# sanderslab/magellanmapper

Measured on AMD Instinct MI355X. Metric: Mvoxels/s, 2048x2048x1024 uint16 stack, 5-sigma LoG blob detection, higher is better.
Workload: dtype f16x2 MFMA (f32 accumulate) + 16-bit fixed-point intermediates; f64 re-score of every candidate

## Files before the change

include/mmx.h:

```cpp
#ifndef MMX_H
#define MMX_H

#include <stddef.h>
#include <stdint.h>

#ifdef __cplusplus
extern "C" {
#endif

#define MMX_ABI_VERSION 21

typedef enum {
    MMX_OK = 0,
    MMX_ERR_ARG = 1,
    MMX_ERR_HIP = 2,
    MMX_ERR_NO_DEVICE = 3,
    MMX_ERR_WORKSPACE = 4,
    MMX_ERR_UNSUPPORTED = 5,
    MMX_DEFERRED = 6
} mmx_status;

typedef enum { MMX_U8 = 0, MMX_U16 = 1, MMX_F32 = 2, MMX_F64 = 3 } mmx_dtype;

#define MMX_MAX_RADIUS_FAST 24
#define MMX_MAX_RADIUS_WIDE 64
#define MMX_MAX_RADIUS_GENERIC 255
#define MMX_MAX_BLOCKS 65535
#define MMX_COLOC_BALL 33

typedef struct {
    int64_t src_off;
    int32_t nz, ny, nx;
    int32_t slot;
    int32_t px;
    int32_t _pad;
} mmx_block;
#define MMX_ROW_ALIGN 32

typedef struct {
    const void* d_data;
    int32_t dtype;
    float value_range;
    int64_t stride_z, stride_y, stride_x;
} mmx_volume;

typedef struct {
    int32_t slot;
    int32_t s;
    int32_t z, y, x;
    uint32_t flags;
    float v;
    float nbr_max;
    double v64;
    uint64_t band;
} mmx_cand;

#define MMX_CAND_CONTESTED 1u
#define MMX_CAND_BAND 2u
#define MMX_CAND_PROBE 4u

int mmx_abi_version(void);
const char* mmx_strerror(int status);
const char* mmx_last_hip_error(void);
int mmx_device_count(void);

typedef enum {
    MMX_ZX_AUTO = -1,
    MMX_ZX_SEPARATE = 0,
    MMX_ZX_PACKED = 2,
    MMX_ZX_TILED = 6,
    MMX_ZX_TILED_Q16 = 7,
    MMX_ZX_WIDE = 8,
    MMX_ZX_THIN = 9
} mmx_zx_mode;
#define MMX_ZX_PREPACKED 0x100
#define MMX_ZX_Y_VALU    0x200
#define MMX_MASK_ROWS 1
#define MMX_MASK_QUADS 2
int mmx_log_batch_f32(const mmx_volume* vol, const mmx_block* d_blocks, const mmx_block* h_blocks,
                      int n_blocks, int64_t slot_elems,
                      const double* h_w0, const double* h_w2, int radius, double norm,
                      float* d_log, float* d_work, uint64_t* d_nms_mask, float nms_lo, float nms_eps,
                      int* h_mask_written, int zx_mode, int* h_zx_path, void* stream);

#define MMX_LOG_ABS_TOL 1e-4

double mmx_tiled_q16_error_bound(const double* h_w0, const double* h_w2, int radius, double norm);

#define MMX_COL_PREFETCH 4
#define MMX_FOLD_MAX_N 68
int mmx_fold_matrix(const float* w, int radius, int n, float* out );
int mmx_col_prefetch(void);

int mmx_zx_pack(const mmx_volume* vol, const mmx_block* d_blocks, const mmx_block* h_blocks, int n_blocks,
                int64_t slot_elems, float* d_work, void* stream);

size_t mmx_workspace_bytes(int n_blocks, int64_t slot_elems, int n_sigma, int with_masks);

int mmx_log_batch_f32_generic(const mmx_volume* vol, const mmx_block* d_blocks,
                              const mmx_block* h_blocks, int n_blocks, int64_t slot_elems,
                              const double* h_w0, const double* h_w2, int radius, double norm,
                              float* d_log, float* d_work, void* stream);

int mmx_peaks_batch(const float* d_log, const uint64_t* d_nms_mask, int mask_layout, int n_sigma, const mmx_block* d_blocks,
                    const mmx_block* h_blocks, int n_blocks, int64_t slot_elems,
                    float thr, float eps, mmx_cand* d_cands, uint32_t cap,
                    uint32_t* d_count, void* stream);

int mmx_rescore_f64(const mmx_volume* vol, const mmx_block* d_blocks, int n_blocks,
                    mmx_cand* d_pts, uint32_t cap, const uint32_t* d_count,
                    const double* d_w0, const double* d_w2, const int32_t* h_radius,
                    const double* h_norm, int n_sigma, int store_f32, void* stream);

int mmx_expand_probes(mmx_cand* d_cands, uint32_t cap, uint32_t* d_count, uint32_t* d_n_cands,
                      const mmx_block* d_blocks, int n_blocks, int n_sigma, void* stream);

typedef struct {
    int32_t parent;
    int32_t off[3];
    int32_t core_lo[3];
    int32_t core_hi[3];
} mmx_part;
int mmx_fold_parts(mmx_cand* d_cands, uint32_t cap, uint32_t* d_count, const mmx_part* d_parts, int n_parts,
                   void* stream);

typedef struct {
    const mmx_volume* vol32;
    const mmx_volume* vol_exact;
    const mmx_block* d_blocks;
    const mmx_block* h_blocks;
    int32_t n_blocks, n_sigma;
    int64_t slot_elems;
    const double* h_w0; const double* h_w2;
    const double* d_w0; const double* d_w2;
    const int32_t* h_radius;
    const double* h_norm;
    float* d_work;
    size_t work_bytes;
    float thr, eps;
    mmx_cand* d_cands;
    uint32_t cap, h_prefix;
    uint32_t* d_count;
    uint32_t* h_count;
    mmx_cand* h_cands;
    int32_t zx_mode, zx_flags, store_f32, exact, expand, _pad;
    void* stream; void* tail_stream; void* pack_stream;
    void* ev_work_free; void* ev_work_read; void* ev_done;
    const mmx_part* d_parts;
    const mmx_block* d_parents;
    const mmx_block* h_parents;
    int32_t n_parts, n_parents;
} mmx_detect_args;
typedef struct {
    int32_t zx_path;
    int32_t mask_layout;
    int32_t n_pass_rounds;
    int32_t _pad;
    double q16_bound;
} mmx_detect_info;
int mmx_detect_batch(const mmx_detect_args* args, mmx_detect_info* info);
const char* mmx_detect_last_error(void);
int mmx_log_scales_f32(const mmx_detect_args* args, mmx_detect_info* info);
int mmx_detect_batch_capture(const mmx_detect_args* args, mmx_detect_info* info, void** graph);
int mmx_graph_launch(void* graph, void* stream, void* ev_done, mmx_detect_info* info);
int mmx_graph_destroy(void* graph);
int mmx_event_synchronize(void* ev);
int mmx_stream_wait_event(void* stream, void* ev);
int mmx_timing_is_enabled(void);

int mmx_overlap_pairs(const double* d_blobs, const int32_t* d_offsets, int n_blocks,
                      double overlap, double band, double max_sigma, int32_t* d_pairs, double* d_frac,
                      uint32_t cap, uint32_t* d_count, void* stream);

int mmx_close_pairs(const int32_t* d_master, int n_master, const int32_t* d_check, int n_check,
                    const int32_t tol[3], int32_t* d_last, uint8_t* d_hit, void* stream);

typedef struct {
    int64_t src_off;
    int64_t dst_off;
    int64_t scratch_off;
    int32_t nz, ny, nx;
    int32_t qclass;
} mmx_subblock;

typedef struct {
    int32_t lo_prev, lo_next, hi_prev, hi_next;
    double lo_gamma, hi_gamma;
} mmx_quantile_class;

typedef struct {
    double clip_min, clip_max;
    double max_thresh;
    double unsharp_strength;
    double erosion_threshold;
    int32_t radius;
    int32_t rgb_guess;
    double tv_weight;
    double tv_factor;
} mmx_preproc_params;

#define MMX_PP_IDENTITY 1
#define MMX_PP_ERODED 2
#define MMX_PP_EXACT_MEAN 4
typedef struct {
    double vmin, vmax, mean;
    int32_t flags;
    int32_t _pad;
} mmx_subblock_info;

#define MMX_PP_RADIUS 32
#define MMX_PP_MAX_SIDE 32
#define MMX_PP_MAX_LDS 163840

int64_t mmx_preprocess_fast_lds(int nz, int ny, int nx);

int mmx_preprocess_batch(const mmx_volume* vol, const mmx_subblock* d_subs, const mmx_subblock* h_subs,
                         int n_subs, const mmx_quantile_class* d_qclasses, int n_qclasses,
                         const mmx_preproc_params* params, const double* d_weights,
                         int64_t dst_sy, int64_t dst_sz, float* d_out32, double* d_out64,
                         mmx_subblock_info* d_info, void* stream);

#define MMX_PP_AUTO 0
#define MMX_PP_SINGLE 1
#define MMX_PP_PIPELINED 2
#define MMX_PP_TILES_PER_WG 8
int64_t mmx_preprocess_work_bytes(const mmx_subblock* h_subs, int n_subs);
int mmx_preprocess_batch_mode(const mmx_volume* vol, const mmx_subblock* d_subs, const mmx_subblock* h_subs,
                              int n_subs, const mmx_quantile_class* d_qclasses, int n_qclasses,
                              const mmx_preproc_params* params, const double* d_weights,
                              int64_t dst_sy, int64_t dst_sz, float* d_out32, double* d_out64,
                              mmx_subblock_info* d_info, int mode, int tiles_per_wg,
                              void* d_work, int64_t work_bytes, void* stream);

int mmx_preprocess_batch_generic(const mmx_volume* vol, const mmx_subblock* d_subs,
                                 const mmx_subblock* h_subs, int n_subs,
                                 const mmx_quantile_class* d_qclasses, int n_qclasses,
                                 const mmx_preproc_params* params, const double* d_weights,
                                 int64_t dst_sy, int64_t dst_sz, float* d_out32, double* d_out64,
                                 mmx_subblock_info* d_info, double* d_scratch, int64_t scratch_doubles,
                                 void* stream);

int mmx_coloc_means(const mmx_volume* vol, const mmx_block* d_blocks, int n_blocks,
                    const int32_t* d_blobs, const int32_t* d_offsets, int n_blobs,
                    double* d_mean, int32_t* d_count, void* stream);
int mmx_coloc_voxels(const mmx_volume* vol, const mmx_block* d_blocks, int n_blocks,
                     const int32_t* d_blobs, const int32_t* d_offsets, int n_blobs,
                     double* d_mean, int32_t* d_count, double* d_voxels, void* stream);

int mmx_unmix_batch(const mmx_volume* vol, const mmx_volume* h_subs, const double* h_facs, int n_subs,
                    const mmx_block* d_blocks, const mmx_block* h_blocks, int n_blocks,
                    int64_t dst_slot, int64_t dst_sy, int64_t dst_sz,
                    float* d_out32, double* d_out64, void* stream);

typedef struct {
    int64_t src_off;
    int32_t in_nz, in_ny, in_nx;
    int32_t out_nz, out_ny, out_nx;
    int32_t slot;
    int32_t tz, ty, tx;
} mmx_resize_block;
int mmx_minmax_batch(const mmx_volume* vol, const mmx_block* d_blocks, const mmx_block* h_blocks,
                     int n_blocks, double* d_minmax, void* stream);
int mmx_resize_batch(const mmx_volume* vol, const mmx_resize_block* d_blocks,
                     const mmx_resize_block* h_blocks, int n_blocks,
                     const int32_t* d_index, const double* d_weight, const double* d_minmax,
                     int64_t dst_slot, int64_t dst_sy, int64_t dst_sz,
                     void* d_out, float* d_out32, void* stream);

int mmx_resize_batch_as(const mmx_volume* vol, const mmx_resize_block* d_blocks,
                        const mmx_resize_block* h_blocks, int n_blocks,
                        const int32_t* d_index, const double* d_weight, const double* d_minmax,
                        int64_t dst_slot, int64_t dst_sy, int64_t dst_sz,
                        int out_dtype, void* d_out, float* d_out32, void* stream);

int mmx_gauss_axis_batch(const mmx_volume* vol, const mmx_block* d_blocks, const mmx_block* h_blocks,
                         int n_blocks, int axis, const double* d_weights, const int32_t* d_radius,
                         int w_pitch, int nearest, int64_t dst_slot, int64_t dst_sy, int64_t dst_sz,
                         void* d_out, void* stream);

typedef struct { int32_t z0, z1; int64_t rank[4]; } mmx_rank_group;
size_t mmx_order_stats_workspace(int n_groups);
int mmx_order_stats(const mmx_volume* vol, int64_t nz, int64_t ny, int64_t nx,
                    const mmx_rank_group* d_groups, const mmx_rank_group* h_groups, int n_groups,
                    double* d_stats , int32_t* d_nan ,
                    void* d_work, size_t work_bytes, void* stream);

#define MMX_K_COUNT 14
#define MMX_K_THIN 14
#define MMX_K_SLOTS 15
int mmx_timing_enable(int on);
int mmx_timing_read(double* ms, int64_t* launches, int n);

int mmx_copy_rect_h2d(void* d_dst, size_t dpitch, const void* h_src, size_t spitch, size_t width, size_t height,
                      void* stream);
int mmx_host_stage_upload(const void* h_src, void* d_dst, const int64_t* regions, int32_t n_regions, int64_t nz,
                          int64_t ny, int64_t row_bytes, void* const* h_staging, int64_t staging_bytes, int32_t depth,
                          void* const* events, void* stream, int32_t device, int64_t* n_queued, const int32_t* cancel,
                          int32_t n_threads);
int mmx_host_stage_upload_pitched(const void* h_src, int64_t src_pitch, void* d_dst, const int64_t* regions,
                                  int32_t n_regions, int64_t nz, int64_t ny, int64_t row_bytes, void* const* h_staging,
                                  int64_t staging_bytes, int32_t depth, void* const* events, void* stream, int32_t device,
                                  int64_t* n_queued, const int32_t* cancel, int32_t n_threads);
int mmx_event_query(void* ev);
int mmx_event_create(void** ev);
int mmx_event_destroy(void* ev);
int mmx_event_record(void* ev, void* stream);
int mmx_event_elapsed_ms(void* start, void* stop, float* ms);

int mmx_host_prune_axis(const int32_t* zyx, const int32_t* tag, double* abs_zyx,
                        const int64_t* cur, int64_t n_cur, int axis, int n_sections,
                        const double* bounds, double last_end, const int32_t tol[3],
                        const double* nxt_lo, const double* nxt_hi,
                        int64_t* out_cur, int64_t* out_n,
                        int64_t* n_slab, int64_t* n_after, int64_t* n_next);

typedef struct {
    const int32_t* src_cols;
    int64_t n_out, n_main;
    int32_t abs_dst[3];
} mmx_row_layout;
int mmx_host_take_rows(const double* table, int64_t ld, const int64_t* rows, int64_t n, const double* abs_zyx,
                       const mmx_row_layout* layout, double* out, double* out_rest);
int mmx_host_gather_parts_by_key(const double* table, int64_t ld, int32_t n_parts, const int64_t* const* ids,
                                 const int64_t* const* keys, const double* const* abs_rows, const int64_t* n_rows,
                                 int64_t n_keys, const mmx_row_layout* layout, double* out, int64_t out_rows,
                                 double* out_rest);

int mmx_host_prune_region(const int32_t* zyx, const int32_t* tag, double* abs_zyx, const int64_t* cur, int64_t n_cur,
                          int64_t own_lo, int64_t own_hi, const int32_t n_sections[3], const double* const bounds[3],
                          const double last_end[3], const int32_t tol[3], const double* const nxt_lo[3],
                          const double* const nxt_hi[3], int64_t* out_rows, int64_t* out_keys, int64_t* out_n,
                          int64_t* n_slab, int64_t* n_after, int64_t* n_next, int64_t stat_ld);
int mmx_host_prune_parts(const int32_t* zyx, const int32_t* tag, const double* abs_zyx, const double* chan,
                         int64_t chan_ld, const int64_t* parts, int n_parts, int own_part, const int32_t box_lo[3],
                         const int32_t box_hi[3], const double* channels, int n_channels,
                         const int32_t n_sections[3], const double* const bounds[3], const double last_end[3],
                         const int32_t tol[3], const double* const nxt_lo[3], const double* const nxt_hi[3],
                         int64_t n_keys, int64_t* out_ids, int64_t* out_keys, double* out_abs, int64_t* out_n,
                         int64_t* n_slab, int64_t* n_after, int64_t* n_next, int64_t stat_ld);
int mmx_host_rows_in_boxes(const int32_t* zyx, const int32_t* tag, const double* abs_zyx, const double* chan,
                           int64_t chan_ld, int64_t n, const int32_t* box_lo, const int32_t* box_hi, int n_boxes,
                           double* out, int64_t cap, int64_t* out_n);
int mmx_host_append_rows(const double* payload, int64_t n, const int32_t lo[3], const int32_t hi[3], int32_t* zyx,
                         int32_t* tag, double* abs_zyx, double* chan, int64_t chan_ld, int64_t at, int64_t cap,
                         int64_t* out_n);
int mmx_host_emit_parts(const double* table, int64_t ld, int32_t n_parts, const int64_t* const* ids,
                        const int64_t* const* keys, const double* const* abs_rows, const int64_t* n_rows,
                        const mmx_row_layout* layout, double* out, int64_t out_rows);
int mmx_host_merge_parts_by_key(const double* const* parts, const int64_t* n_rows, int32_t n_parts, int64_t ld,
                                int64_t n_keys, int64_t n_cols, double* out, int64_t out_rows);

int mmx_host_map_columns(const double* table, int64_t ld, int64_t n, const int32_t* src_cols,
                         int32_t n_map, double* out, int64_t out_ld, int32_t dst_col0);

int mmx_host_resolve_peaks(const mmx_cand* cands, uint32_t n_cands, uint32_t n_total, const mmx_block* blocks,
                           int n_blocks, int n_sigma, double thr, int32_t* out_nz_coords, double* out_nz_vals,
                           int32_t* out_coords, double* out_vals, int32_t* offsets, uint8_t* ties, double* stats);
int mmx_host_overlap_prune(const int32_t* coords, const int32_t* offsets, int n_blocks, const double* sigmas,
                           int n_sigma, double overlap, double band, uint8_t* alive, uint8_t* open_blocks,
                           int32_t* pairs, double* frac, int64_t cap, int64_t* n_pairs, int64_t* n_knife);
int mmx_host_emit_tables(const int32_t* coords, const uint8_t* alive, const int32_t* offsets, int n_blocks,
                         const double* sigmas, int n_sigma, double channel, const double* block_offsets,
                         const int32_t* block_tags, const int32_t* interior, double* store, int64_t ld,
                         int32_t* zyx, int32_t* tag, double* abs_zyx, int64_t row0, int64_t capacity,
                         int64_t* rows_per_block);
int mmx_host_emit_tables_multi(int32_t n_channels, const int32_t* const* coords, const uint8_t* const* alive,
                               const int32_t* const* offsets, int n_blocks, const double* const* sigmas,
                               const int32_t* n_sigma, const double* channel_ids, const double* block_offsets,
                               const int32_t* block_tags, const int32_t* interior, double* store, int64_t ld,
                               int32_t n_extra, int32_t* zyx, int32_t* tag, double* abs_zyx, int64_t row0,
                               int64_t capacity, int64_t* rows_per_block, uint8_t* any_before, int32_t* coloc_rows);
int mmx_host_coloc_flags(const double* means, const int32_t* mean_channels, int32_t n_mean_channels, int64_t n,
                         const int32_t* rows, const int64_t* row_offsets, int n_blocks, const int32_t* shapes,
                         int32_t n_channels, double* flags, int64_t ld);

typedef struct {
    const mmx_cand* cands; uint32_t n_cands, n_total;
    const mmx_block* blocks; int32_t n_blocks, n_sigma;
    double thr, eps;
    const double* sigmas; double overlap, overlap_band;
    double channel;
    const double* block_offsets; const int32_t* block_tags; const int32_t* interior;
    double* store; int64_t ld; int32_t* zyx; int32_t* tag; double* abs_zyx; int64_t capacity;
    int64_t* rows_per_block; uint8_t* any_before;
    const int32_t* n_sections; const double* const* bounds; const double* last_end; const int32_t* tol;
    const double* const* nxt_lo; const double* const* nxt_hi;
    int64_t* n_slab; int64_t* n_after; int64_t* n_next; int64_t stat_ld;
    const int32_t* src_cols; int32_t n_out, abs_dst0;
    double* out; int64_t out_capacity; int64_t* out_rows;
    double* stats;
} mmx_finish_stack_args;
int mmx_host_finish_stack(const mmx_finish_stack_args* a);

int mmx_cdist_f64(const double* d_a, int64_t n, const double* d_b, int64_t m, int dim, double* d_out, void* stream);
int mmx_host_lsap(const double* cost, int64_t nr, int64_t nc, int64_t* out_rows, int64_t* out_cols);

#define MMX_PATCH_MAX_SIZE 4096
int mmx_extract_patches(const mmx_volume* vol, const int32_t* d_zyx, int64_t n, int size, void* d_out, float* d_out32,
                        void* stream);

int mmx_calib_stream(int kind, const void* d_in, void* d_out, int64_t n_elems, void* stream);

#ifdef __cplusplus
}
#endif
#endif
```

magellanmapper_amd/_native.py:

```python
from __future__ import annotations

import ctypes
import os
from ctypes import (POINTER, Structure, c_char_p, c_double, c_float, c_int, c_int32, c_int64,
                    c_uint8, c_uint32, c_void_p)

import numpy as np

_HERE = os.path.dirname(os.path.abspath(__file__))
LIB_PATH = os.environ.get("MMX_LIB_PATH") or os.path.join(_HERE, "libmmx_hip.so")

MMX_ABI_VERSION = 21
MMX_U8, MMX_U16, MMX_F32, MMX_F64 = 0, 1, 2, 3
MMX_MAX_RADIUS_FAST = 24
MMX_MAX_RADIUS_WIDE = 64
MMX_MAX_RADIUS_GENERIC = 255
MMX_CAND_CONTESTED = 1
MMX_CAND_BAND = 2
MMX_CAND_PROBE = 4
MMX_ZX_AUTO, MMX_ZX_SEPARATE, MMX_ZX_PACKED, MMX_ZX_MFMA_F32, MMX_ZX_MFMA_F16, MMX_ZX_MFMA_F16_LDS = -1, 0, 2, 3, 4, 5
MMX_ZX_TILED, MMX_ZX_TILED_Q16, MMX_ZX_PREPACKED, MMX_ZX_Y_VALU = 6, 7, 0x100, 0x200
MMX_ZX_WIDE = 8
MMX_ZX_THIN = 9
MMX_FOLD_MAX_N = 68
MMX_MASK_ROWS, MMX_MASK_QUADS = 1, 2
MMX_MAX_BLOCKS = 65535
MMX_COLOC_BALL = 33
MMX_PATCH_MAX_SIZE = 4096

BLOCK_DTYPE = np.dtype([("src_off", "<i8"), ("nz", "<i4"), ("ny", "<i4"), ("nx", "<i4"),
                        ("slot", "<i4"), ("px", "<i4"), ("_pad", "<i4")], align=True)
MMX_ROW_ALIGN = 32
CAND_DTYPE = np.dtype([("slot", "<i4"), ("s", "<i4"), ("z", "<i4"), ("y", "<i4"), ("x", "<i4"),
                       ("flags", "<u4"), ("v", "<f4"), ("nbr_max", "<f4"), ("v64", "<f8"),
                       ("band", "<u8")], align=True)
assert BLOCK_DTYPE.itemsize == 32 and CAND_DTYPE.itemsize == 48
PART_DTYPE = np.dtype([("parent", "<i4"), ("off", "<i4", (3,)), ("core_lo", "<i4", (3,)), ("core_hi", "<i4", (3,))],
                      align=True)
assert PART_DTYPE.itemsize == 40
SUBBLOCK_DTYPE = np.dtype([("src_off", "<i8"), ("dst_off", "<i8"), ("scratch_off", "<i8"),
                           ("nz", "<i4"), ("ny", "<i4"), ("nx", "<i4"), ("qclass", "<i4")], align=True)
QCLASS_DTYPE = np.dtype([("lo_prev", "<i4"), ("lo_next", "<i4"), ("hi_prev", "<i4"), ("hi_next", "<i4"),
                         ("lo_gamma", "<f8"), ("hi_gamma", "<f8")], align=True)
SUBINFO_DTYPE = np.dtype([("vmin", "<f8"), ("vmax", "<f8"), ("mean", "<f8"), ("flags", "<i4"),
                          ("_pad", "<i4")], align=True)
assert SUBBLOCK_DTYPE.itemsize == 40 and QCLASS_DTYPE.itemsize == 32 and SUBINFO_DTYPE.itemsize == 32
MMX_PP_IDENTITY, MMX_PP_ERODED, MMX_PP_EXACT_MEAN = 1, 2, 4
MMX_PP_AUTO, MMX_PP_SINGLE, MMX_PP_PIPELINED = 0, 1, 2
RESIZE_DTYPE = np.dtype([("src_off", "<i8"), ("in_nz", "<i4"), ("in_ny", "<i4"), ("in_nx", "<i4"),
                         ("out_nz", "<i4"), ("out_ny", "<i4"), ("out_nx", "<i4"), ("slot", "<i4"),
                         ("tz", "<i4"), ("ty", "<i4"), ("tx", "<i4")], align=True)
assert RESIZE_DTYPE.itemsize == 48
RANK_GROUP_DTYPE = np.dtype([("z0", "<i4"), ("z1", "<i4"), ("rank", "<i8", (4,))], align=True)
assert RANK_GROUP_DTYPE.itemsize == 40


class Volume(Structure):
    _fields_ = [("d_data", c_void_p), ("dtype", c_int32), ("value_range", c_float),
                ("stride_z", c_int64), ("stride_y", c_int64), ("stride_x", c_int64)]


class DetectArgs(Structure):
    _fields_ = [("vol32", POINTER(Volume)), ("vol_exact", POINTER(Volume)), ("d_blocks", c_void_p),
                ("h_blocks", c_void_p), ("n_blocks", c_int32), ("n_sigma", c_int32), ("slot_elems", c_int64),
                ("h_w0", c_void_p), ("h_w2", c_void_p), ("d_w0", c_void_p), ("d_w2", c_void_p),
                ("h_radius", c_void_p), ("h_norm", c_void_p), ("d_work", c_void_p), ("work_bytes", ctypes.c_size_t),
                ("thr", c_float), ("eps", c_float), ("d_cands", c_void_p), ("cap", c_uint32), ("h_prefix", c_uint32),
                ("d_count", c_void_p), ("h_count", c_void_p), ("h_cands", c_void_p),
                ("zx_mode", c_int32), ("zx_flags", c_int32), ("store_f32", c_int32), ("exact", c_int32),
                ("expand", c_int32), ("_pad", c_int32),
                ("stream", c_void_p), ("tail_stream", c_void_p), ("pack_stream", c_void_p),
                ("ev_work_free", c_void_p), ("ev_work_read", c_void_p), ("ev_done", c_void_p),
                ("d_parts", c_void_p), ("d_parents", c_void_p), ("h_parents", c_void_p),
                ("n_parts", c_int32), ("n_parents", c_int32)]


class FinishStackArgs(Structure):
    _fields_ = [("cands", c_void_p), ("n_cands", c_uint32), ("n_total", c_uint32),
                ("blocks", c_void_p), ("n_blocks", c_int32), ("n_sigma", c_int32),
                ("thr", c_double), ("eps", c_double),
                ("sigmas", c_void_p), ("overlap", c_double), ("overlap_band", c_double),
                ("channel", c_double),
                ("block_offsets", c_void_p), ("block_tags", c_void_p), ("interior", c_void_p),
                ("store", c_void_p), ("ld", c_int64), ("zyx", c_void_p), ("tag", c_void_p), ("abs_zyx", c_void_p),
                ("capacity", c_int64), ("rows_per_block", c_void_p), ("any_before", c_void_p),
                ("n_sections", c_void_p), ("bounds", c_void_p), ("last_end", c_void_p), ("tol", c_void_p),
                ("nxt_lo", c_void_p), ("nxt_hi", c_void_p),
                ("n_slab", c_void_p), ("n_after", c_void_p), ("n_next", c_void_p), ("stat_ld", c_int64),
                ("src_cols", c_void_p), ("n_out", c_int32), ("abs_dst0", c_int32),
                ("out", c_void_p), ("out_capacity", c_int64), ("out_rows", c_void_p),
                ("stats", c_void_p)]


MMX_DEFERRED = 6


class RowLayout(Structure):
    _fields_ = [("src_cols", POINTER(c_int32)), ("n_out", c_int64), ("n_main", c_int64), ("abs_dst", c_int32 * 3)]


class DetectInfo(Structure):
    _fields_ = [("zx_path", c_int32), ("mask_layout", c_int32), ("n_pass_rounds", c_int32), ("_pad", c_int32),
                ("q16_bound", c_double)]


class PreprocParams(Structure):
    _fields_ = [("clip_min", c_double), ("clip_max", c_double), ("max_thresh", c_double),
                ("unsharp_strength", c_double), ("erosion_threshold", c_double),
                ("radius", c_int32), ("rgb_guess", c_int32), ("tv_weight", c_double), ("tv_factor", c_double)]


class MmxError(RuntimeError):
    """A C-ABI call returned a non-zero status."""


_lib = None

SYMBOLS = (
    "mmx_abi_version", "mmx_strerror", "mmx_last_hip_error", "mmx_device_count",
    "mmx_detect_batch", "mmx_log_scales_f32", "mmx_detect_batch_capture", "mmx_graph_launch", "mmx_graph_destroy", "mmx_detect_last_error",
    "mmx_event_synchronize", "mmx_stream_wait_event", "mmx_timing_is_enabled",
    "mmx_log_batch_f32", "mmx_log_batch_f32_generic", "mmx_zx_pack", "mmx_fold_matrix", "mmx_col_prefetch", "mmx_tiled_q16_error_bound", "mmx_workspace_bytes", "mmx_peaks_batch", "mmx_rescore_f64",
    "mmx_overlap_pairs", "mmx_close_pairs", "mmx_event_create", "mmx_event_destroy",
    "mmx_event_record", "mmx_event_elapsed_ms", "mmx_timing_enable", "mmx_timing_read",
    "mmx_calib_stream", "mmx_host_prune_axis",
    "mmx_preprocess_fast_lds", "mmx_preprocess_batch", "mmx_preprocess_batch_mode", "mmx_preprocess_work_bytes", "mmx_preprocess_batch_generic",
    "mmx_coloc_means", "mmx_coloc_voxels", "mmx_host_take_rows", "mmx_host_map_columns", "mmx_resize_batch_as", "mmx_gauss_axis_batch", "mmx_unmix_batch", "mmx_minmax_batch", "mmx_resize_batch",
    "mmx_cdist_f64", "mmx_host_lsap", "mmx_expand_probes", "mmx_fold_parts", "mmx_host_resolve_peaks", "mmx_host_overlap_prune",
    "mmx_host_emit_tables", "mmx_host_prune_region", "mmx_host_prune_parts", "mmx_host_rows_in_boxes", "mmx_host_append_rows", "mmx_host_emit_parts", "mmx_host_merge_parts_by_key", "mmx_host_gather_parts_by_key", "mmx_host_emit_tables_multi", "mmx_host_coloc_flags", "mmx_host_finish_stack", "mmx_copy_rect_h2d", "mmx_host_stage_upload", "mmx_host_stage_upload_pitched", "mmx_event_query",
    "mmx_order_stats_workspace", "mmx_order_stats", "mmx_extract_patches",
)
KERNEL_KINDS = ("zpass", "ypass", "xpass", "generic", "peaks", "rescore", "overlap_pairs",
                "close_pairs", "zxpass", "y2pass", "preproc", "coloc", "zxpack", "widepass")
MORE_KERNEL_KINDS = ("thinpass",)
_ALL_KINDS = KERNEL_KINDS + MORE_KERNEL_KINDS


def lib() -> ctypes.CDLL:
    global _lib
    if _lib is not None:
        return _lib
    if not os.path.exists(LIB_PATH):
        raise MmxError(
            f"{LIB_PATH} not found: the HIP extension has not been built "
            "(run __graft_entry__.build() or make -C magellanmapper_amd/csrc). "
            "There is no CPU fallback for this path.")
    try:
        import torch
    except ImportError:
        pass
    L = ctypes.CDLL(LIB_PATH)
    missing = [name for name in SYMBOLS if not hasattr(L, name)]
    if missing:
        raise MmxError(f"{LIB_PATH} lacks {', '.join(missing)}: it was built from older sources; rebuild it")
    vp = c_void_p
    L.mmx_abi_version.restype = c_int
    L.mmx_strerror.restype = c_char_p
    L.mmx_strerror.argtypes = [c_int]
    L.mmx_last_hip_error.restype = c_char_p
    L.mmx_device_count.restype = c_int
    log_args = [POINTER(Volume), vp, vp, c_int, c_int64, POINTER(c_double), POINTER(c_double),
                c_int, c_double, vp, vp]
    L.mmx_log_batch_f32.argtypes = log_args + [vp, c_float, c_float, POINTER(c_int), c_int, POINTER(c_int), vp]
    L.mmx_log_batch_f32_generic.argtypes = log_args + [vp]
    L.mmx_workspace_bytes.argtypes = [c_int, c_int64, c_int, c_int]
    L.mmx_workspace_bytes.restype = ctypes.c_size_t
    L.mmx_zx_pack.argtypes = [POINTER(Volume), vp, vp, c_int, c_int64, vp, vp]
    L.mmx_tiled_q16_error_bound.argtypes = [POINTER(c_double), POINTER(c_double), c_int, c_double]
    L.mmx_tiled_q16_error_bound.restype = c_double
    L.mmx_fold_matrix.argtypes = [POINTER(c_float), c_int, c_int, POINTER(c_float)]
    L.mmx_fold_matrix.restype = c_int
    L.mmx_col_prefetch.argtypes = []
    L.mmx_col_prefetch.restype = c_int
    L.mmx_peaks_batch.argtypes = [vp, vp, c_int, c_int, vp, vp, c_int, c_int64, c_float, c_float, vp,
                                  c_uint32, vp, vp]
    L.mmx_rescore_f64.argtypes = [POINTER(Volume), vp, c_int, vp, c_uint32, vp, vp, vp,
                                  POINTER(c_int32), POINTER(c_double), c_int, c_int, vp]
    L.mmx_overlap_pairs.argtypes = [vp, vp, c_int, c_double, c_double, c_double, vp, vp, c_uint32, vp, vp]
    L.mmx_close_pairs.argtypes = [vp, c_int, vp, c_int, POINTER(c_int32), vp, vp, vp]
    L.mmx_detect_batch.argtypes = [POINTER(DetectArgs), POINTER(DetectInfo)]
    L.mmx_log_scales_f32.argtypes = [POINTER(DetectArgs), POINTER(DetectInfo)]
    L.mmx_detect_batch_capture.argtypes = [POINTER(DetectArgs), POINTER(DetectInfo), POINTER(vp)]
    L.mmx_graph_launch.argtypes = [vp, vp, vp, POINTER(DetectInfo)]
    L.mmx_graph_destroy.argtypes = [vp]
    L.mmx_detect_last_error.restype = c_char_p
    L.mmx_event_synchronize.argtypes = [vp]
    L.mmx_stream_wait_event.argtypes = [vp, vp]
    L.mmx_event_create.argtypes = [POINTER(vp)]
    L.mmx_event_destroy.argtypes = [vp]
    L.mmx_event_record.argtypes = [vp, vp]
    L.mmx_event_elapsed_ms.argtypes = [vp, vp, POINTER(c_float)]
    L.mmx_timing_enable.argtypes = [c_int]
    L.mmx_timing_read.argtypes = [POINTER(c_double), POINTER(c_int64), c_int]
    L.mmx_calib_stream.argtypes = [c_int, vp, vp, c_int64, vp]
    L.mmx_host_prune_axis.argtypes = [vp, vp, vp, vp, c_int64, c_int, c_int, vp, c_double,
                                      POINTER(c_int32), vp, vp, vp, POINTER(c_int64), vp, vp, vp]
    L.mmx_preprocess_fast_lds.argtypes = [c_int, c_int, c_int]
    L.mmx_preprocess_fast_lds.restype = c_int64
    pre_args = [POINTER(Volume), vp, vp, c_int, vp, c_int, POINTER(PreprocParams), vp,
                c_int64, c_int64, vp, vp, vp]
    L.mmx_preprocess_batch.argtypes = pre_args + [vp]
    L.mmx_preprocess_batch_mode.argtypes = pre_args + [c_int, c_int, vp, c_int64, vp]
    L.mmx_preprocess_work_bytes.argtypes = [vp, c_int]
    L.mmx_preprocess_work_bytes.restype = c_int64
    L.mmx_preprocess_batch_generic.argtypes = pre_args + [vp, c_int64, vp]
    L.mmx_minmax_batch.argtypes = [POINTER(Volume), vp, vp, c_int, vp, vp]
    L.mmx_minmax_batch.restype = c_int
    L.mmx_resize_batch.argtypes = [POINTER(Volume), vp, vp, c_int, vp, vp, vp, c_int64, c_int64, c_int64,
                                   vp, vp, vp]
    L.mmx_resize_batch.restype = c_int
    L.mmx_resize_batch_as.argtypes = [POINTER(Volume), vp, vp, c_int, vp, vp, vp, c_int64, c_int64, c_int64,
                                      c_int, vp, vp, vp]
    L.mmx_resize_batch_as.restype = c_int
    L.mmx_gauss_axis_batch.argtypes = [POINTER(Volume), vp, vp, c_int, c_int, vp, vp, c_int, c_int,
                                       c_int64, c_int64, c_int64, vp, vp]
    L.mmx_gauss_axis_batch.restype = c_int
    L.mmx_unmix_batch.argtypes = [POINTER(Volume), POINTER(Volume), POINTER(c_double), c_int, vp, vp, c_int,
                                  c_int64, c_int64, c_int64, vp, vp, vp]
    L.mmx_unmix_batch.restype = c_int
    L.mmx_host_take_rows.argtypes = [vp, c_int64, vp, c_int64, vp, POINTER(RowLayout), vp, vp]
    L.mmx_host_map_columns.argtypes = [vp, c_int64, c_int64, POINTER(c_int32), c_int32, vp, c_int64, c_int32]
    L.mmx_cdist_f64.argtypes = [vp, c_int64, vp, c_int64, c_int, vp, vp]
    L.mmx_cdist_f64.restype = c_int
    L.mmx_host_lsap.argtypes = [vp, c_int64, c_int64, vp, vp]
    L.mmx_host_lsap.restype = c_int
    L.mmx_coloc_means.argtypes = [POINTER(Volume), vp, c_int, vp, vp, c_int, vp, vp, vp]
    L.mmx_coloc_means.restype = c_int
    L.mmx_coloc_voxels.argtypes = [POINTER(Volume), vp, c_int, vp, vp, c_int, vp, vp, vp, vp]
    L.mmx_coloc_voxels.restype = c_int
    L.mmx_expand_probes.argtypes = [vp, c_uint32, vp, vp, vp, c_int, c_int, vp]
    L.mmx_expand_probes.restype = c_int
    L.mmx_fold_parts.argtypes = [vp, c_uint32, vp, vp, c_int, vp]
    L.mmx_fold_parts.restype = c_int
    L.mmx_host_resolve_peaks.argtypes = [vp, c_uint32, c_uint32, vp, c_int, c_int, c_double, vp, vp, vp, vp, vp, vp, vp]
    L.mmx_host_overlap_prune.argtypes = [vp, vp, c_int, vp, c_int, c_double, c_double, vp, vp, vp, vp, c_int64,
                                         POINTER(c_int64), POINTER(c_int64)]
    L.mmx_host_prune_region.argtypes = [vp, vp, vp, vp, c_int64, c_int64, c_int64, POINTER(c_int32), POINTER(vp),
                                        POINTER(c_double), POINTER(c_int32), POINTER(vp), POINTER(vp), vp, vp,
                                        POINTER(c_int64), vp, vp, vp, c_int64]
    L.mmx_host_prune_parts.argtypes = [vp, vp, vp, vp, c_int64, vp, c_int, c_int, POINTER(c_int32), POINTER(c_int32),
                                       vp, c_int, POINTER(c_int32), POINTER(vp), POINTER(c_double), POINTER(c_int32),
                                       POINTER(vp), POINTER(vp), c_int64, vp, vp, vp, POINTER(c_int64), vp, vp, vp,
                                       c_int64]
    L.mmx_host_rows_in_boxes.argtypes = [vp, vp, vp, vp, c_int64, c_int64, vp, vp, c_int, vp, c_int64, POINTER(c_int64)]
    L.mmx_host_append_rows.argtypes = [vp, c_int64, POINTER(c_int32), POINTER(c_int32), vp, vp, vp, vp, c_int64,
                                       c_int64, c_int64, POINTER(c_int64)]
    L.mmx_host_gather_parts_by_key.argtypes = [vp, c_int64, c_int32, vp, vp, vp, vp, c_int64, POINTER(RowLayout), vp, c_int64, vp]
    L.mmx_host_emit_parts.argtypes = [vp, c_int64, c_int32, vp, vp, vp, vp, POINTER(RowLayout), vp, c_int64]
    L.mmx_host_merge_parts_by_key.argtypes = [vp, vp, c_int32, c_int64, c_int64, c_int64, vp, c_int64]
    L.mmx_host_emit_tables_multi.argtypes = [c_int32, vp, vp, vp, c_int, vp, vp, vp, vp, vp, vp, vp, c_int64, c_int32, vp, vp,
                                             vp, c_int64, c_int64, vp, vp, vp]
    L.mmx_host_coloc_flags.argtypes = [vp, vp, c_int32, c_int64, vp, vp, c_int, vp, c_int32, vp, c_int64]
    L.mmx_host_finish_stack.argtypes = [POINTER(FinishStackArgs)]
    L.mmx_host_stage_upload.argtypes = [vp, vp, vp, c_int32, c_int64, c_int64, c_int64, vp, c_int64, c_int32, vp, vp, c_int32,
                                        vp, vp, c_int32]
    L.mmx_host_stage_upload_pitched.argtypes = [vp, c_int64, vp, vp, c_int32, c_int64, c_int64, c_int64, vp, c_int64, c_int32,
                                                vp, vp, c_int32, vp, vp, c_int32]
    L.mmx_event_query.argtypes = [vp]
    L.mmx_copy_rect_h2d.argtypes = [vp, ctypes.c_size_t, vp, ctypes.c_size_t, ctypes.c_size_t, ctypes.c_size_t, vp]
    L.mmx_host_emit_tables.argtypes = [vp, vp, vp, c_int, vp, c_int, c_double, vp, vp, vp, vp, c_int64, vp, vp, vp,
                                       c_int64, c_int64, vp]
    L.mmx_order_stats_workspace.argtypes = [c_int]
    L.mmx_order_stats_workspace.restype = ctypes.c_size_t
    L.mmx_order_stats.argtypes = [POINTER(Volume), c_int64, c_int64, c_int64, vp, vp, c_int, vp, vp, vp, ctypes.c_size_t, vp]
    L.mmx_order_stats.restype = c_int
    L.mmx_extract_patches.argtypes = [POINTER(Volume), vp, c_int64, c_int, vp, vp, vp]
    L.mmx_extract_patches.restype = c_int
    L.mmx_preprocess_batch.restype = c_int
    L.mmx_preprocess_batch_mode.restype = c_int
    L.mmx_preprocess_batch_generic.restype = c_int
    for name in SYMBOLS:
        fn = getattr(L, name)
        if name in ("mmx_preprocess_fast_lds", "mmx_workspace_bytes", "mmx_preprocess_work_bytes",
                    "mmx_order_stats_workspace"):
            continue
        if fn.restype is None or name.startswith(("mmx_log", "mmx_peaks", "mmx_rescore",
                                                  "mmx_overlap", "mmx_close", "mmx_event", "mmx_timing", "mmx_calib", "mmx_host")):
            fn.restype = c_int
    if L.mmx_abi_version() != MMX_ABI_VERSION:
        raise MmxError("libmmx_hip.so ABI version mismatch")
    _lib = L
    return L


def check(status: int, what: str) -> None:
    if status != 0:
        L = lib()
        msg = L.mmx_strerror(status).decode()
        hip = L.mmx_last_hip_error().decode()
        raise MmxError(f"{what}: {msg}" + (f" ({hip})" if hip else ""))


def as_double_ptr(a: np.ndarray):
    assert a.dtype == np.float64 and a.flags.c_contiguous
    return a.ctypes.data_as(POINTER(c_double))


def as_int32_ptr(a: np.ndarray):
    assert a.dtype == np.int32 and a.flags.c_contiguous
    return a.ctypes.data_as(POINTER(c_int32))


def timing_enable(on: bool = True, kinds=None) -> None:
    mask = 1 if on else 0
    if on and kinds is not None:
        mask = 0
        for k in kinds:
            mask |= 1 << (_ALL_KINDS.index(k) + 1)
    check(lib().mmx_timing_enable(mask), "mmx_timing_enable")


def timing_read() -> dict:
    ms = (c_double * len(_ALL_KINDS))()
    n = (c_int64 * len(_ALL_KINDS))()
    check(lib().mmx_timing_read(ms, n, len(_ALL_KINDS)), "mmx_timing_read")
    return {k: (ms[i], n[i]) for i, k in enumerate(_ALL_KINDS)}


def col_prefetch() -> int:
    return int(lib().mmx_col_prefetch())


def fold_matrix(w: np.ndarray, n: int) -> np.ndarray:
    w = np.ascontiguousarray(w, dtype=np.float32)
    out = np.empty((int(n), int(n)), dtype=np.float32)
    check(lib().mmx_fold_matrix(w.ctypes.data_as(POINTER(c_float)), len(w) - 1, int(n),
                                out.ctypes.data_as(POINTER(c_float))), "mmx_fold_matrix")
    return out


def keep_host_heap(mmap_threshold: int = 1 << 30, trim_threshold: int = (1 << 31) - 1) -> bool:
    try:
        libc = ctypes.CDLL("libc.so.6")
        ok1 = libc.mallopt(-3, int(mmap_threshold))
        ok2 = libc.mallopt(-1, int(trim_threshold))
        return bool(ok1 and ok2)
    except (OSError, AttributeError):
        return False
```

magellanmapper_amd/csrc/mmx_api.hip:

```cpp

#include <atomic>
#include <cstdio>
#include <cstdlib>
#include <cstring>

#include "mmx_common.h"

int mmx_launch_generic_pass(int pass, const mmx_volume* vol, const mmx_block* d_blocks, int n_blocks,
                            int max_vox, int64_t slot_elems, const float* w0, const float* w2, int radius,
                            const float* in1, const float* in2, float* out1, float* out2, hipStream_t s);
int mmx_launch_fold_pass(int pass, const mmx_volume* vol, const mmx_block* d_blocks, int n_blocks,
                         int max_vox, int64_t slot_elems, const float* w0, const float* w2, int radius,
                         const float* in1, const float* in2, float* out1, float* out2, hipStream_t s);
int mmx_launch_peaks(const float* d_log, int n_sigma, int64_t sigma_stride, const mmx_block* d_blocks,
                     int n_blocks, int max_vox, int64_t slot_elems, float thr, float eps,
                     mmx_cand* d_cands, uint32_t cap, uint32_t* d_count, hipStream_t stream);
int mmx_launch_peaks_sparse(const float* d_log, const unsigned long long* d_mask, int n_sigma,
                            int64_t sigma_stride, const mmx_block* d_blocks, int n_blocks, int max_vox,
                            int64_t slot_elems, float thr, float eps, mmx_cand* d_cands, uint32_t cap,
                            uint32_t* d_count, int quads, hipStream_t stream);

#include <mutex>
#include <vector>

namespace {
thread_local char g_hip_err[256] = "";

struct span { hipEvent_t a, b; int kind; };
std::mutex g_tm;
bool g_timing = false;
uint32_t g_kinds = ~0u;
std::vector<span> g_spans;
std::vector<hipEvent_t> g_pool;
hipEvent_t g_open[MMX_K_SLOTS];

hipEvent_t take_event()
{
    if (!g_pool.empty()) { hipEvent_t e = g_pool.back(); g_pool.pop_back(); return e; }
    hipEvent_t e = nullptr;
    hipEventCreate(&e);
    return e;
}

int hip_fail(hipError_t e, const char* what)
{
    snprintf(g_hip_err, sizeof g_hip_err, "%s: %s", what, hipGetErrorString(e));
    return MMX_ERR_HIP;
}
}

void mmx_time_begin(int kind, hipStream_t s)
{
    std::lock_guard<std::mutex> lk(g_tm);
    if (!g_timing || !((g_kinds >> kind) & 1u)) return;
    g_open[kind] = take_event();
    hipEventRecord(g_open[kind], s);
}

void mmx_time_end(int kind, hipStream_t s)
{
    std::lock_guard<std::mutex> lk(g_tm);
    if (!g_timing || !g_open[kind]) return;
    hipEvent_t b = take_event();
    hipEventRecord(b, s);
    g_spans.push_back({g_open[kind], b, kind});
    g_open[kind] = nullptr;
}

extern "C" {

int mmx_timing_enable(int on)
{
    std::lock_guard<std::mutex> lk(g_tm);
    for (auto& sp : g_spans) { g_pool.push_back(sp.a); g_pool.push_back(sp.b); }
    g_spans.clear();
    for (int k = 0; k < MMX_K_SLOTS; ++k) g_open[k] = nullptr;
    g_timing = on != 0;
    g_kinds = on == 1 ? ~0u : ((uint32_t)on >> 1);
    return MMX_OK;
}

int mmx_timing_is_enabled(void)
{
    std::lock_guard<std::mutex> lk(g_tm);
    return g_timing ? 1 : 0;
}

int mmx_timing_read(double* ms, int64_t* launches, int n)
{
    if (!ms || !launches || n < MMX_K_COUNT) return MMX_ERR_ARG;
    std::lock_guard<std::mutex> lk(g_tm);
    for (int k = 0; k < n; ++k) { ms[k] = 0.0; launches[k] = 0; }
    for (auto& sp : g_spans) {
        if (sp.kind >= n) {
            g_pool.push_back(sp.a);
            g_pool.push_back(sp.b);
            continue;
        }
        hipError_t r = hipEventSynchronize(sp.b);
        if (r != hipSuccess) return hip_fail(r, "hipEventSynchronize");
        float t = 0.f;
        r = hipEventElapsedTime(&t, sp.a, sp.b);
        if (r != hipSuccess) return hip_fail(r, "hipEventElapsedTime");
        ms[sp.kind] += t;
        launches[sp.kind] += 1;
        g_pool.push_back(sp.a);
        g_pool.push_back(sp.b);
    }
    g_spans.clear();
    return MMX_OK;
}

int mmx_abi_version(void) { return MMX_ABI_VERSION; }
size_t mmx_workspace_bytes(int n_blocks, int64_t slot_elems, int n_sigma, int with_masks)
{
    if (n_blocks < 1 || slot_elems < 1 || n_sigma < 1) return 0;
    size_t bytes = (size_t)(4 + n_sigma) * (size_t)n_blocks * (size_t)slot_elems * sizeof(float);
    if (with_masks) {
        bytes = (bytes + 15) & ~(size_t)15;
        bytes += (size_t)n_sigma * (((size_t)n_blocks * (size_t)slot_elems) >> 5) * 16;
    }
    return bytes;
}

const char* mmx_strerror(int status)
{
    switch (status) {
        case MMX_OK: return "ok";
        case MMX_ERR_ARG: return "bad argument";
        case MMX_ERR_HIP: return "HIP runtime error";
        case MMX_ERR_NO_DEVICE: return "no gfx950 device";
        case MMX_ERR_WORKSPACE: return "workspace too small";
        case MMX_ERR_UNSUPPORTED: return "unsupported configuration";
        case MMX_DEFERRED: return "left to the caller";
        default: return "unknown status";
    }
}

const char* mmx_last_hip_error(void) { return g_hip_err; }


int mmx_device_count(void)
{
    int n = 0;
    hipError_t e = hipGetDeviceCount(&n);
    if (e != hipSuccess) { hip_fail(e, "hipGetDeviceCount"); return -1; }
    int ok = 0;
    for (int i = 0; i < n; ++i) {
        hipDeviceProp_t p;
        if (hipGetDeviceProperties(&p, i) == hipSuccess && strncmp(p.gcnArchName, "gfx950", 6) == 0) ++ok;
    }
    return ok;
}

double mmx_tiled_q16_error_bound(const double* h_w0, const double* h_w2, int radius, double norm)
{
    return mmx_q16_error_bound(h_w0, h_w2, radius, norm);
}

}

void mmx_batch_geom_make(const mmx_volume* vol, const mmx_block* h_blocks, int n_blocks, int64_t slot_elems,
                         mmx_batch_geom* g)
{
    *g = mmx_batch_geom{};
    g->min_nz = g->min_ny = g->min_nx = 1 << 30;
    g->plan_status = MMX_ERR_UNSUPPORTED;
    g->rows_fit = g->quads_fit = true;
    if (n_blocks < 1 || n_blocks > MMX_MAX_BLOCKS) {
        g->status = n_blocks < 1 ? MMX_ERR_ARG : MMX_ERR_UNSUPPORTED;
        return;
    }
    for (int i = 0; i < n_blocks; ++i) {
        const mmx_block& b = h_blocks[i];
        if (b.nz < 1 || b.ny < 1 || b.nx < 1 || b.slot != i || b.px < b.nx || b.px % MMX_ROW_ALIGN) {
            if (g->status == MMX_OK) g->status = MMX_ERR_ARG;
            g->bad_block = true;
            return;
        }
        if ((int64_t)b.nz * b.ny * b.px > slot_elems && g->status == MMX_OK) g->status = MMX_ERR_WORKSPACE;
        if (b.nz < g->min_nz) g->min_nz = b.nz;
        if (b.ny < g->min_ny) g->min_ny = b.ny;
        if (b.nx < g->min_nx) g->min_nx = b.nx;
        if (b.ny > g->max_ny) g->max_ny = b.ny;
        if (b.nx > g->max_nx) g->max_nx = b.nx;
        if (b.px > g->max_px) g->max_px = b.px;
        if (b.ny * b.px > g->max_zcols) g->max_zcols = b.ny * b.px;
        if (b.nz * b.px > g->max_ycols) g->max_ycols = b.nz * b.px;
        if (b.nz * b.ny > g->max_rows) g->max_rows = b.nz * b.ny;
        if (b.nz * b.ny * b.px > g->max_vox) g->max_vox = b.nz * b.ny * b.px;
        if (!mmx_entries_fit(MMX_MASK_ROWS, b.nz, b.ny, b.nx, b.px, slot_elems)) g->rows_fit = false;
        if (!mmx_entries_fit(MMX_MASK_QUADS, b.nz, b.ny, b.nx, b.px, slot_elems)) g->quads_fit = false;
        if (vol) {
            const int64_t lane = (int64_t)(b.ny - 1) * vol->stride_y + (int64_t)(b.nx - 1) * vol->stride_x;
            if (lane > g->max_lane_in) g->max_lane_in = lane;
        }
    }
    if (vol) g->plan_status = mmx_zx6_plan_make(h_blocks, n_blocks, slot_elems, vol->dtype, &g->plan);
}

namespace {

struct pass_weights {
    float z0[MMX_MAX_RADIUS_GENERIC + 1], z2[MMX_MAX_RADIUS_GENERIC + 1];
    float y0[MMX_MAX_RADIUS_GENERIC + 1], y2[MMX_MAX_RADIUS_GENERIC + 1];
    float x0[MMX_MAX_RADIUS_GENERIC + 1], x2[MMX_MAX_RADIUS_GENERIC + 1];
};
void make_weights(const mmx_volume* vol, const double* h_w0, const double* h_w2, int radius, double norm, pass_weights* w)
{
    double in_scale = 1.0;
    if (vol->dtype == MMX_U8) in_scale = 1.0 / 255.0;
    else if (vol->dtype == MMX_U16) in_scale = 1.0 / 65535.0;
    for (int k = 0; k <= radius; ++k) {
        w->z0[k] = (float)(h_w0[k] * in_scale);
        w->z2[k] = (float)(h_w2[k] * in_scale);
        w->y0[k] = (float)h_w0[k];
        w->y2[k] = (float)h_w2[k];
        w->x0[k] = (float)(-norm * h_w0[k]);
        w->x2[k] = (float)(-norm * h_w2[k]);
    }
}
mmx_taps_f32 taps(const float* a, const float* b, int radius)
{
    mmx_taps_f32 t;
    for (int k = 0; k <= MMX_MAX_RADIUS_FAST; ++k) {
        t.w0[k] = k <= radius ? a[k] : 0.f;
        t.w2[k] = k <= radius ? b[k] : 0.f;
    }
    return t;
}

int launched(int rc, const char* launcher, const char* what)
{
    if (rc == MMX_ERR_HIP) return hip_fail(hipGetLastError(), what);
    if (rc == MMX_ERR_UNSUPPORTED) {
        char msg[128];
        snprintf(msg, sizeof msg, "%s refused a call its route accepted", launcher);
        mmx_detect_set_error(msg);
    }
    return rc;
}

struct pass_scope {
    int kind; hipStream_t s;
    pass_scope(int k, hipStream_t st) : kind(k), s(st) { if (k >= 0) mmx_time_begin(k, st); }
    ~pass_scope() { if (kind >= 0) mmx_time_end(kind, s); }
};

int fused_passes(const mmx_log_call& c, const mmx_route& r, const mmx_batch_geom& g, const pass_weights& w)
{
    const mmx_volume* vol = c.vol;
    const int radius = c.radius, n_blocks = c.n_blocks;
    const int64_t slot_elems = c.slot_elems;
    hipStream_t s = c.stream;
    float* t0 = c.d_work;
    float* t1 = c.d_work + (int64_t)n_blocks * slot_elems;
    mmx_taps_f32 tzz = taps(w.z0, w.z2, radius), txx = taps(w.y0, w.y2, radius), tyy = taps(w.x0, w.x2, radius);
    const bool tiled = r.family == MMX_ROUTE_TILED;
    const mmx_zx6_plan& plan = g.plan;
    int rc;
    if (r.makes_copy) {
        mmx_timed_scope ts(MMX_K_ZXPACK, s);
        rc = mmx_launch_zx6_pack(vol, c.d_blocks, c.h_blocks, n_blocks, plan, c.d_work, s);
        if (rc != MMX_OK) return launched(rc, "mmx_launch_zx6_pack", "voxel copy of the tiled path");
    }
    { mmx_timed_scope ts(MMX_K_ZX, s);
      if (tiled)
          rc = mmx_launch_zx6(vol, c.d_blocks, c.h_blocks, n_blocks, plan, txx, radius, c.d_work,
                              r.q16 ? (float)(1.0 / r.bp) : 0.f, r.q16 ? (float)(1.0 / r.bq) : 0.f, s);
      else
          rc = mmx_launch_zx2(vol, c.d_blocks, n_blocks, g.max_ny, g.max_px, slot_elems, tzz, txx, radius, t0, t1, s); }
    if (rc != MMX_OK) return launched(rc, tiled ? "mmx_launch_zx6" : "mmx_launch_zx2", "fused passes");
    { mmx_timed_scope ts(MMX_K_Y2, s);
      unsigned long long* d_mask = r.layout ? (unsigned long long*)c.d_nms_mask : nullptr;
      const float cp = r.q16 ? (float)(r.bp / 65535.0) : 0.f, cq = r.q16 ? (float)(r.bq / 32767.0) : 0.f;
      if (r.y_kernel == MMX_Y_YM)
          rc = mmx_launch_ym(c.d_blocks, n_blocks, plan, slot_elems, tyy, radius, c.d_work, cp, cq, c.d_log, d_mask,
                             c.nms_lo, c.nms_eps, s);
      else if (r.y_kernel == MMX_Y_Y6)
          rc = mmx_launch_y6(c.d_blocks, n_blocks, plan, slot_elems, tyy, radius, c.d_work,
                             reinterpret_cast<const float*>(reinterpret_cast<const char*>(c.d_work) + plan.q_off), cp, cq,
                             c.d_log, d_mask, c.nms_lo, c.nms_eps, s);
      else
          rc = mmx_launch_y2(c.d_blocks, n_blocks, g.max_ycols, slot_elems, tyy, radius, t0, t1, c.d_log, d_mask, c.nms_lo,
                             c.nms_eps, s); }
    return launched(rc, r.y_kernel == MMX_Y_YM ? "mmx_launch_ym" : (r.y_kernel == MMX_Y_Y6 ? "mmx_launch_y6" : "mmx_launch_y2"),
                    "fused passes");
}

int wide_passes(const mmx_log_call& c, const mmx_route& r, const pass_weights& w)
{
    const int radius = c.radius, n_blocks = c.n_blocks;
    const int64_t slot_elems = c.slot_elems;
    hipStream_t s = c.stream;
    float* t0 = c.d_work;
    float* t1 = t0 + (int64_t)n_blocks * slot_elems;
    float* t2 = t1 + (int64_t)n_blocks * slot_elems;
    float* t3 = t2 + (int64_t)n_blocks * slot_elems;
    unsigned long long* d_mask = r.layout ? (unsigned long long*)c.d_nms_mask : nullptr;
    int rc;
    { mmx_timed_scope ts(MMX_K_WIDE, s);
      rc = mmx_launch_wide_pass(0, c.vol, c.d_blocks, c.h_blocks, n_blocks, slot_elems, w.z0, w.z2, radius, nullptr, nullptr,
                                t2, t3, nullptr, 0.f, 0.f, s); }
    if (rc == MMX_OK) {
        mmx_timed_scope ts(MMX_K_WIDE, s);
        rc = mmx_launch_wide_pass(1, c.vol, c.d_blocks, c.h_blocks, n_blocks, slot_elems, w.y0, w.y2, radius, t2, t3, t0, t1,
                                  nullptr, 0.f, 0.f, s);
    }
    if (rc == MMX_OK) {
        mmx_timed_scope ts(MMX_K_WIDE, s);
        rc = mmx_launch_wide_pass(2, c.vol, c.d_blocks, c.h_blocks, n_blocks, slot_elems, w.x0, w.x2, radius, t0, t1, c.d_log,
                                  nullptr, d_mask, c.nms_lo, c.nms_eps, s);
    }
    return launched(rc, "mmx_launch_wide_pass", "wide passes");
}

int three_passes(const mmx_volume* vol, const mmx_block* d_blocks, int n_blocks, int64_t slot_elems, int radius,
                 float* d_work, float* d_log, const mmx_batch_geom& g, const pass_weights& w, int rings, int folds,
                 bool timed, hipStream_t s)
{
    float* t0 = d_work;
    float* t1 = t0 + (int64_t)n_blocks * slot_elems;
    float* t2 = t1 + (int64_t)n_blocks * slot_elems;
    float* t3 = t2 + (int64_t)n_blocks * slot_elems;
    const float* w0[3] = {w.z0, w.y0, w.x0};
    const float* w2[3] = {w.z2, w.y2, w.x2};
    const float* in1[3] = {nullptr, t0, t2};
    const float* in2[3] = {nullptr, t1, t3};
    float* out1[3] = {t0, t2, d_log};
    float* out2[3] = {t1, t3, nullptr};
    const int ring_kind[3] = {MMX_K_ZPASS, MMX_K_YPASS, MMX_K_XPASS};
    const char* ring_name[3] = {"mmx_launch_zpass", "mmx_launch_ypass", "mmx_launch_xpass"};
    const char* what[3] = {"z pass", "y pass", "x pass"};
    for (int p = 0; p < 3; ++p) {
        const bool ring = (rings >> p) & 1, fold = !ring && ((folds >> p) & 1);
        int rc;
        { pass_scope ts(!timed ? -1 : (ring ? ring_kind[p] : (fold ? MMX_K_THIN : MMX_K_GENERIC)), s);
        if (ring && p == 0) rc = mmx_launch_zpass(vol, d_blocks, n_blocks, g.max_zcols, slot_elems, taps(w.z0, w.z2, radius), radius, t0, t1, s);
        else if (ring && p == 1) rc = mmx_launch_ypass(d_blocks, n_blocks, g.max_ycols, slot_elems, taps(w.y0, w.y2, radius), radius, t0, t1, t2, t3, s);
        else if (ring) rc = mmx_launch_xpass(d_blocks, n_blocks, g.max_rows, g.max_nx, slot_elems, taps(w.x0, w.x2, radius), radius, t2, t3, d_log, s);
        else rc = (fold ? mmx_launch_fold_pass : mmx_launch_generic_pass)(p, vol, d_blocks, n_blocks, g.max_vox, slot_elems, w0[p], w2[p],
                                                                          radius, in1[p], in2[p], out1[p], out2[p], s); }
        if (rc != MMX_OK)
            return launched(rc, ring ? ring_name[p] : (fold ? "mmx_launch_fold_pass" : "mmx_launch_generic_pass"), what[p]);
    }
    return MMX_OK;
}

}

int mmx_log_scale_check(const mmx_log_call& c)
{
    mmx_zx_request q;
    if (mmx_zx_parse(c.zx_mode, &q) != MMX_OK) return MMX_ERR_ARG;
    if (!c.vol || !c.vol->d_data || !c.d_blocks || !c.h_blocks || !c.h_w0 || !c.h_w2 || !c.d_log || !c.d_work)
        return MMX_ERR_ARG;
    if (c.n_blocks < 1 || c.radius < 0 || c.slot_elems < 1) return MMX_ERR_ARG;
    if (c.n_blocks > MMX_MAX_BLOCKS) return MMX_ERR_UNSUPPORTED;
    if (c.radius > MMX_MAX_RADIUS_GENERIC) return MMX_ERR_UNSUPPORTED;
    if (c.slot_elems >= (int64_t(1) << 29)) return MMX_ERR_UNSUPPORTED;
    if (c.slot_elems % MMX_ROW_ALIGN) return MMX_ERR_ARG;
    if (!mmx_voxels_ok(c.vol)) return MMX_ERR_UNSUPPORTED;
    return MMX_OK;
}

int mmx_log_scale_run(const mmx_log_call& c, const mmx_batch_geom& g, const mmx_route& r)
{
    pass_weights w;
    make_weights(c.vol, c.h_w0, c.h_w2, c.radius, c.norm, &w);
    int rc;
    if (r.family == MMX_ROUTE_WIDE) rc = wide_passes(c, r, w);
    else if (r.family == MMX_ROUTE_SEPARATE)
        rc = three_passes(c.vol, c.d_blocks, c.n_blocks, c.slot_elems, c.radius, c.d_work, c.d_log, g, w,
                          r.ring_z | r.ring_y << 1 | r.ring_x << 2, r.fold_z | r.fold_y << 1 | r.fold_x << 2, true, c.stream);
    else rc = fused_passes(c, r, g, w);
    if (rc != MMX_OK) return rc;
    if (c.h_zx_path) *c.h_zx_path = r.path;
    if (c.h_mask_written) *c.h_mask_written = r.layout;
    return MMX_OK;
}

namespace {
int log_scale(const mmx_log_call& c, const mmx_batch_geom& g)
{
    if (c.h_mask_written) *c.h_mask_written = 0;
    if (c.h_zx_path) *c.h_zx_path = MMX_ZX_SEPARATE;
    int rc = mmx_log_scale_check(c);
    if (rc != MMX_OK) return rc;
    mmx_route r;
    rc = mmx_route_scale(c.vol, g, c.radius, c.h_w0, c.h_w2, c.norm, c.zx_mode, c.nms_eps, c.d_nms_mask && c.h_mask_written, &r);
    return rc != MMX_OK ? rc : mmx_log_scale_run(c, g, r);
}
}

int mmx_zx_pack_geom(const mmx_volume* vol, const mmx_block* d_blocks, const mmx_block* h_blocks, int n_blocks,
                     int64_t slot_elems, const mmx_batch_geom& g, float* d_work, hipStream_t stream)
{
    if (!vol || !vol->d_data || !d_blocks || !h_blocks || !d_work || n_blocks < 1 || slot_elems < 1) return MMX_ERR_ARG;
    if (n_blocks > MMX_MAX_BLOCKS) return MMX_ERR_UNSUPPORTED;
    if (vol->dtype != MMX_U8 && vol->dtype != MMX_U16 && vol->dtype != MMX_F32) return MMX_ERR_UNSUPPORTED;
    if (g.bad_block) return MMX_ERR_ARG;
    if (g.plan_status != MMX_OK) return g.plan_status;
    mmx_timed_scope ts(MMX_K_ZXPACK, stream);
    const int rc = mmx_launch_zx6_pack(vol, d_blocks, h_blocks, n_blocks, g.plan, d_work, stream);
    return rc == MMX_ERR_HIP ? hip_fail(hipGetLastError(), "voxel copy of the tiled path") : rc;
}

extern "C" {

int mmx_log_batch_f32(const mmx_volume* vol, const mmx_block* d_blocks, const mmx_block* h_blocks,
                      int n_blocks, int64_t slot_elems,
                      const double* h_w0, const double* h_w2, int radius, double norm,
                      float* d_log, float* d_work, uint64_t* d_nms_mask, float nms_lo, float nms_eps,
                      int* h_mask_written, int zx_mode, int* h_zx_path, void* stream)
{
    mmx_batch_geom g{};
    if (vol && h_blocks) mmx_batch_geom_make(vol, h_blocks, n_blocks, slot_elems, &g);
    return log_scale({vol, d_blocks, h_blocks, n_blocks, slot_elems, h_w0, h_w2, radius, norm, d_log, d_work,
                              d_nms_mask, nms_lo, nms_eps, h_mask_written, zx_mode, h_zx_path, (hipStream_t)stream}, g);
}

int mmx_log_batch_f32_generic(const mmx_volume* vol, const mmx_block* d_blocks, const mmx_block* h_blocks,
                              int n_blocks, int64_t slot_elems,
                              const double* h_w0, const double* h_w2, int radius, double norm,
                              float* d_log, float* d_work, void* stream)
{
    if (!vol || !vol->d_data || !d_blocks || !h_blocks || !h_w0 || !h_w2 || !d_log || !d_work)
        return MMX_ERR_ARG;
    if (n_blocks < 1 || radius < 0 || radius > MMX_MAX_RADIUS_GENERIC || slot_elems < 1) return MMX_ERR_ARG;
    if (n_blocks > MMX_MAX_BLOCKS) return MMX_ERR_UNSUPPORTED;
    mmx_batch_geom g;
    mmx_batch_geom_make(vol, h_blocks, n_blocks, slot_elems, &g);
    if (g.status != MMX_OK) return g.status;
    pass_weights w;
    make_weights(vol, h_w0, h_w2, radius, norm, &w);
    return three_passes(vol, d_blocks, n_blocks, slot_elems, radius, d_work, d_log, g, w, 0, 0, false, (hipStream_t)stream);
}

int mmx_zx_pack(const mmx_volume* vol, const mmx_block* d_blocks, const mmx_block* h_blocks, int n_blocks,
                int64_t slot_elems, float* d_work, void* stream)
{
    mmx_batch_geom g{};
    if (vol && h_blocks) mmx_batch_geom_make(vol, h_blocks, n_blocks, slot_elems, &g);
    return mmx_zx_pack_geom(vol, d_blocks, h_blocks, n_blocks, slot_elems, g, d_work, (hipStream_t)stream);
}

int mmx_peaks_batch(const float* d_log, const uint64_t* d_nms_mask, int mask_layout, int n_sigma, const mmx_block* d_blocks,
                    const mmx_block* h_blocks, int n_blocks, int64_t slot_elems,
                    float thr, float eps, mmx_cand* d_cands, uint32_t cap,
                    uint32_t* d_count, void* stream)
{
    if (!d_log || !d_blocks || !h_blocks || !d_cands || !d_count) return MMX_ERR_ARG;
    if (n_sigma < 1 || n_blocks < 1 || slot_elems < 1 || !(eps >= 0.f)) return MMX_ERR_ARG;
    if (n_blocks > MMX_MAX_BLOCKS) return MMX_ERR_UNSUPPORTED;
    if (slot_elems % MMX_ROW_ALIGN) return MMX_ERR_ARG;
    if (d_nms_mask && mask_layout != MMX_MASK_ROWS && mask_layout != MMX_MASK_QUADS) return MMX_ERR_ARG;
    mmx_batch_geom g;
    mmx_batch_geom_make(nullptr, h_blocks, n_blocks, slot_elems, &g);
    if (g.status != MMX_OK) return g.status;
    const int max_vox = g.max_vox;
    mmx_timed_scope ts(MMX_K_PEAKS, (hipStream_t)stream);
    int rc;
    if (d_nms_mask)
        rc = mmx_launch_peaks_sparse(d_log, (const unsigned long long*)d_nms_mask, n_sigma,
                                     (int64_t)n_blocks * slot_elems, d_blocks, n_blocks, max_vox, slot_elems,
                                     thr, eps, d_cands, cap, d_count, mask_layout == MMX_MASK_QUADS, (hipStream_t)stream);
    else
        rc = mmx_launch_peaks(d_log, n_sigma, (int64_t)n_blocks * slot_elems, d_blocks, n_blocks, max_vox,
                              slot_elems, thr, eps, d_cands, cap, d_count, (hipStream_t)stream);
    return rc == MMX_ERR_HIP ? hip_fail(hipGetLastError(), "peaks") : rc;
}

int mmx_copy_rect_h2d(void* d_dst, size_t dpitch, const void* h_src, size_t spitch, size_t width, size_t height,
                      void* stream)
{
    if (!d_dst || !h_src || width > dpitch || width > spitch) return MMX_ERR_ARG;
    if (!width || !height) return MMX_OK;
    hipError_t r = hipMemcpy2DAsync(d_dst, dpitch, h_src, spitch, width, height, hipMemcpyHostToDevice, (hipStream_t)stream);
    return r == hipSuccess ? MMX_OK : hip_fail(r, "hipMemcpy2DAsync");
}

int mmx_event_create(void** ev)
{
    if (!ev) return MMX_ERR_ARG;
    hipEvent_t e;
    hipError_t r = hipEventCreate(&e);
    if (r != hipSuccess) return hip_fail(r, "hipEventCreate");
    *ev = (void*)e;
    return MMX_OK;
}

int mmx_event_destroy(void* ev)
{
    hipError_t r = hipEventDestroy((hipEvent_t)ev);
    return r == hipSuccess ? MMX_OK : hip_fail(r, "hipEventDestroy");
}

int mmx_event_record(void* ev, void* stream)
{
    hipError_t r = hipEventRecord((hipEvent_t)ev, (hipStream_t)stream);
    return r == hipSuccess ? MMX_OK : hip_fail(r, "hipEventRecord");
}

int mmx_event_elapsed_ms(void* start, void* stop, float* ms)
{
    if (!ms) return MMX_ERR_ARG;
    hipError_t r = hipEventSynchronize((hipEvent_t)stop);
    if (r != hipSuccess) return hip_fail(r, "hipEventSynchronize");
    r = hipEventElapsedTime(ms, (hipEvent_t)start, (hipEvent_t)stop);
    return r == hipSuccess ? MMX_OK : hip_fail(r, "hipEventElapsedTime");
}

}
```

magellanmapper_amd/csrc/mmx_common.h:

```cpp
#pragma once

#include <hip/hip_runtime.h>
#include <stdint.h>

#include "../../include/mmx.h"

#define MMX_WG 256
#define MMX_MAX_GRID_X 2147483647

struct mmx_taps_f32 {
    float w0[MMX_MAX_RADIUS_FAST + 1];
    float w2[MMX_MAX_RADIUS_FAST + 1];
};

__host__ __device__ __forceinline__ int mmx_reflect(int i, int n)
{
    if (n == 1) return 0;
    const int period = 2 * n;
    i %= period;
    if (i < 0) i += period;
    return i < n ? i : period - 1 - i;
}

int mmx_launch_zpass(const mmx_volume* vol, const mmx_block* d_blocks, int n_blocks, int max_cols,
                     int64_t slot_elems, const mmx_taps_f32& taps, int radius,
                     float* d_gz, float* d_gzz, hipStream_t stream);
int mmx_launch_ypass(const mmx_block* d_blocks, int n_blocks, int max_cols, int64_t slot_elems,
                     const mmx_taps_f32& taps, int radius, const float* d_gz, const float* d_gzz,
                     float* d_a, float* d_bc, hipStream_t stream);
int mmx_launch_xpass(const mmx_block* d_blocks, int n_blocks, int max_rows, int max_nx,
                     int64_t slot_elems, const mmx_taps_f32& taps, int radius,
                     const float* d_a, const float* d_bc, float* d_log, hipStream_t stream);

int mmx_launch_zx2(const mmx_volume* vol, const mmx_block* d_blocks, int n_blocks, int max_ny, int max_px,
                   int64_t slot_elems, const mmx_taps_f32& tz, const mmx_taps_f32& tx, int radius,
                   float* d_p, float* d_q, hipStream_t s);
struct mmx_zx6_plan {
    int64_t tile_stride;
    int64_t pack_stride;
    int64_t q_off, tab_off, pack_off;
    int64_t tab_bytes;
    int max_tiles;
    int max_rowtiles;
};
int mmx_zx6_plan_make(const mmx_block* h_blocks, int n_blocks, int64_t slot_elems, int voxel_dtype, mmx_zx6_plan* plan);
int mmx_launch_zx6_pack(const mmx_volume* vol, const mmx_block* d_blocks, const mmx_block* h_blocks, int n_blocks,
                        const mmx_zx6_plan& plan, void* d_work, hipStream_t stream);
int mmx_launch_zx6(const mmx_volume* vol, const mmx_block* d_blocks, const mmx_block* h_blocks, int n_blocks,
                   const mmx_zx6_plan& plan, const mmx_taps_f32& tx, int radius, void* d_work, float qp, float qq,
                   hipStream_t stream);
int mmx_launch_y6(const mmx_block* d_blocks, int n_blocks, const mmx_zx6_plan& plan, int64_t slot_elems,
                  const mmx_taps_f32& taps, int radius, const float* d_p, const float* d_q, float cp, float cq,
                  float* d_log, unsigned long long* d_mask, float nms_lo, float nms_eps, hipStream_t stream);
int mmx_launch_ym(const mmx_block* d_blocks, int n_blocks, const mmx_zx6_plan& plan, int64_t slot_elems,
                  const mmx_taps_f32& taps, int radius, const float* d_p, float cp, float cq,
                  float* d_log, unsigned long long* d_mask, float nms_lo, float nms_eps, hipStream_t stream);
int mmx_launch_y2(const mmx_block* d_blocks, int n_blocks, int max_cols, int64_t slot_elems,
                  const mmx_taps_f32& taps, int radius, const float* d_p, const float* d_q,
                  float* d_log, unsigned long long* d_mask, float nms_lo, float nms_eps, hipStream_t stream);

int mmx_launch_wide_pass(int pass, const mmx_volume* vol, const mmx_block* d_blocks, const mmx_block* h_blocks, int n_blocks,
                         int64_t slot_elems, const float* w0, const float* w2, int radius,
                         const float* in1, const float* in2, float* out1, float* out2,
                         unsigned long long* d_mask, float nms_lo, float nms_eps, hipStream_t s);

struct mmx_batch_geom {
    int status;
    bool bad_block;
    int min_nz, min_ny, min_nx, max_ny, max_nx, max_px;
    int max_zcols, max_ycols, max_rows, max_vox;
    int64_t max_lane_in;
    bool rows_fit, quads_fit;
    mmx_zx6_plan plan;
    int plan_status;
};
void mmx_batch_geom_make(const mmx_volume* vol, const mmx_block* h_blocks, int n_blocks, int64_t slot_elems, mmx_batch_geom* g);

#include "mmx_entries.h"

#include "mmx_route.h"

struct mmx_log_call {
    const mmx_volume* vol; const mmx_block* d_blocks; const mmx_block* h_blocks; int n_blocks; int64_t slot_elems;
    const double* h_w0; const double* h_w2; int radius; double norm;
    float* d_log; float* d_work; uint64_t* d_nms_mask; float nms_lo, nms_eps; int* h_mask_written;
    int zx_mode; int* h_zx_path; hipStream_t stream;
};
int mmx_log_scale_check(const mmx_log_call& c);
int mmx_log_scale_run(const mmx_log_call& c, const mmx_batch_geom& g, const mmx_route& r);
int mmx_zx_pack_geom(const mmx_volume* vol, const mmx_block* d_blocks, const mmx_block* h_blocks, int n_blocks,
                     int64_t slot_elems, const mmx_batch_geom& g, float* d_work, hipStream_t stream);
void mmx_detect_set_error(const char* msg);

enum mmx_kernel_kind {
    MMX_K_ZPASS = 0, MMX_K_YPASS, MMX_K_XPASS, MMX_K_GENERIC, MMX_K_PEAKS, MMX_K_RESCORE,
    MMX_K_PAIRS, MMX_K_CLOSE, MMX_K_ZX, MMX_K_Y2, MMX_K_PREPROC, MMX_K_COLOC, MMX_K_ZXPACK, MMX_K_WIDE, MMX_K_END
};
void mmx_time_begin(int kind, hipStream_t s);
void mmx_time_end(int kind, hipStream_t s);
static_assert(MMX_K_END == MMX_K_COUNT, "kernel kinds out of sync with mmx.h");
static_assert(MMX_K_THIN == MMX_K_END && MMX_K_SLOTS == MMX_K_THIN + 1, "the thin family follows the counted ones");
struct mmx_timed_scope {
    int kind; hipStream_t s;
    mmx_timed_scope(int k, hipStream_t st) : kind(k), s(st) { mmx_time_begin(k, st); }
    ~mmx_timed_scope() { mmx_time_end(kind, s); }
};
```

magellanmapper_amd/csrc/mmx_fused4.hip:

```cpp

#include <algorithm>
#include <type_traits>

#include "mmx_device.h"

#define MMX_ZX4_MAXCLS 8
#ifndef ZX4_ST_AUX
#define ZX4_ST_AUX 0
#endif
#ifndef ZX4_LD_AUX
#define ZX4_LD_AUX 0
#endif

struct mmx_zx4_cfg {
    float w0[MMX_MAX_RADIUS_FAST + 1];
    float w2[MMX_MAX_RADIUS_FAST + 1];
    float xscale;
    int radius;
    int ncw, ncz;
    int wcls[MMX_ZX4_MAXCLS];
    int zcls[MMX_ZX4_MAXCLS];
    int maxcol, maxu;
    float qp, qq;
    int staged;
    int ntw;
};

namespace {

#ifndef ZX4_PF
#define ZX4_PF 3
#endif
constexpr int kPF4 = ZX4_PF;
#ifndef ZX6_PF
#define ZX6_PF 2
#endif
constexpr float kLoScale = 2048.f;
constexpr float kLoInv = 1.f / 2048.f;

template <int NKX, int LA> struct cls4 {
    static constexpr int R8 = NKX == 1 ? 8 : (LA == 1 ? 16 : 24);
    static __host__ __device__ constexpr int xstart(int c)
    {
        const int lo = 16 * c - R8;
        const int al = lo & ~31;
        return (al + 32 * NKX >= 16 * c + 16 + R8) ? al : lo;
    }
    static constexpr bool SPLIT = LA == 2;
    static constexpr int NKZ = 2;
    static constexpr int NT = 4;
};

__device__ __forceinline__ float folded_tap(const float* w, int R, int p, int o, int n)
{
    float s = 0.f;
    int d = p - o; d = d < 0 ? -d : d;
    if (d <= R) s += w[d];
    d = (-1 - p) - o; d = d < 0 ? -d : d;
    if (d <= R) s += w[d];
    d = (2 * n - 1 - p) - o; d = d < 0 ? -d : d;
    if (d <= R) s += w[d];
    return s;
}

template <int NKX, int LA>
__global__ void __launch_bounds__(256)
zx4_setup(mmx_zx4_cfg cfg, v4u* __restrict__ xtab, v4u* __restrict__ ztab)
{
    using cg = cls4<NKX, LA>;
    const int R = cfg.radius;
    const int lane = threadIdx.x & 63;
    const int kq = lane >> 4, col = lane & 15;
    const int e = blockIdx.x * 4 + (threadIdx.x >> 6);
    const int nx_entries = cfg.ncw * cfg.maxcol * NKX * 2;
    const int nz_entries = cfg.ncz * cfg.maxu * cg::NKZ * 2;
    float wt[8];
    v4u* dst;
    if (e < nx_entries) {
        const int kern = e & 1;
        const int m = (e >> 1) % NKX;
        const int c = ((e >> 1) / NKX) % cfg.maxcol;
        const int cl = ((e >> 1) / NKX) / cfg.maxcol;
        const int W = cfg.wcls[cl];
        const float* w = kern ? cfg.w2 : cfg.w0;
        const int xo = 16 * c + col;
        const int cwin = cfg.ntw == 2 ? (c & ~1) : c;
        const int xc = (cfg.staged == 2 ? 16 * cwin - cg::R8 : cg::xstart(c)) + 32 * m + 8 * kq;
        int xl = xc < 0 ? 0 : xc;
        xl = xl > W - 8 ? W - 8 : xl;
        if (cfg.staged) xl = xc;
#pragma unroll
        for (int j = 0; j < 8; ++j) {
            const int p = xl + j;
            const bool ok = p >= xc && p < xc + 8 && p >= 0 && p < W && xo < W;
            wt[j] = ok ? folded_tap(w, R, p, xo, W) * cfg.xscale * (cfg.qp > 0.f ? (kern ? cfg.qq : cfg.qp) : 1.f) : 0.f;
        }
        dst = xtab + (size_t)e * 2 * 64;
    } else if (e < nx_entries + nz_entries) {
        const int ez = e - nx_entries;
        const int kern = ez & 1;
        const int ks = (ez >> 1) % cg::NKZ;
        const int U = ((ez >> 1) / cg::NKZ) % cfg.maxu;
        const int cl = ((ez >> 1) / cg::NKZ) / cfg.maxu;
        const int nz = cfg.zcls[cl];
        const float* w = kern ? cfg.w2 : cfg.w0;
        const int zo = 16 * U + col;
#pragma unroll
        for (int j = 0; j < 8; ++j) {
            const int i = 2 * ks + (j >> 2);
            const int tile = cg::SPLIT ? (i == 0 ? (kq < 2 ? U + 2 : U - 2) : U - 2 + i) : U - LA + i;
            const int zi = 16 * tile + 4 * kq + (j & 3);
            const bool ok = (cg::SPLIT || i < cg::NT - 1) && zi >= 0 && zi < nz && zo < nz;
            wt[j] = ok ? folded_tap(w, R, zi, zo, nz) * (cfg.qp > 0.f && kern ? cfg.qq / cfg.qp : 1.f) : 0.f;
        }
        dst = ztab + (size_t)ez * 2 * 64;
    } else {
        return;
    }
    unsigned hi[4], lo[4];
#pragma unroll
    for (int j = 0; j < 8; j += 2) {
        const v2f v = {wt[j], wt[j + 1]};
        const v2h h = __builtin_convertvector(v, v2h);
        const v2f r = {(wt[j] - (float)h.x) * kLoScale, (wt[j + 1] - (float)h.y) * kLoScale};
        hi[j >> 1] = __builtin_bit_cast(unsigned, h);
        lo[j >> 1] = __builtin_bit_cast(unsigned, __builtin_convertvector(r, v2h));
    }
    dst[lane] = (v4u){hi[0], hi[1], hi[2], hi[3]};
    dst[64 + lane] = (v4u){lo[0], lo[1], lo[2], lo[3]};
}

template <typename InT> struct pieces4;
template <> struct pieces4<uint16_t> {
    using raw_t = v4u;
    static __device__ __forceinline__ raw_t load(rsrc_t r, unsigned off, unsigned soff = 0)
    {
        return __builtin_bit_cast(v4u, __builtin_amdgcn_raw_buffer_load_b128(r, off, soff, ZX4_LD_AUX));
    }
    static __device__ __forceinline__ void split(const raw_t& d, v4u& hi, v4u& lo)
    {
        const v2h four = {(_Float16)4.0f, (_Float16)4.0f};
        const v2h sixty4th = {(_Float16)0.015625f, (_Float16)0.015625f};
#pragma unroll
        for (int i = 0; i < 4; ++i) {
            const unsigned th = __builtin_amdgcn_perm(0x44004400u, d[i], 0x07030501u);
            const unsigned tl = __builtin_amdgcn_perm(0x24002400u, d[i], 0x07020500u);
            hi[i] = __builtin_bit_cast(unsigned, __builtin_bit_cast(v2h, th) - four);
            lo[i] = __builtin_bit_cast(unsigned, __builtin_bit_cast(v2h, tl) - sixty4th);
        }
    }
    static constexpr float kBiasHi = 4.0f, kBiasLo = 0.015625f;
    static __device__ __forceinline__ void split_biased(const raw_t& d, v4u& hi, v4u& lo)
    {
#pragma unroll
        for (int i = 0; i < 4; ++i) {
            hi[i] = __builtin_amdgcn_perm(0x44004400u, d[i], 0x07030501u);
            lo[i] = __builtin_amdgcn_perm(0x24002400u, d[i], 0x07020500u);
        }
    }
};

struct presplit_t { v4u h, l; };
template <> struct pieces4<float> {
    using raw_t = presplit_t;
    static __device__ __forceinline__ raw_t load(rsrc_t r, unsigned off, unsigned soff = 0)
    {
        raw_t v;
        v.h = __builtin_bit_cast(v4u, __builtin_amdgcn_raw_buffer_load_b128(r, off, soff, ZX4_LD_AUX));
        v.l = __builtin_bit_cast(v4u, __builtin_amdgcn_raw_buffer_load_b128(r, off + 256u, soff, ZX4_LD_AUX));
        return v;
    }
    static __device__ __forceinline__ void split(const raw_t& d, v4u& hi, v4u& lo) { hi = d.h; lo = d.l; }
    [[maybe_unused]] static constexpr float kBiasHi = 0.f, kBiasLo = 0.f;
    static __device__ __forceinline__ void split_biased(const raw_t& d, v4u& hi, v4u& lo) { hi = d.h; lo = d.l; }
};
template <typename InT> struct is_f32_4 { static constexpr bool value = false; };
template <> struct is_f32_4<float> { static constexpr bool value = true; };
template <typename InT> struct lo_scaled4 { static constexpr bool value = false; };
template <> struct lo_scaled4<float> { static constexpr bool value = true; };

template <int NKX, int LA, typename InT, bool Q16 = false, int NTW = 1>
__global__ void __launch_bounds__(256, (NTW == 1 && (LA == 1 || Q16) && !is_f32_4<InT>::value) ? 3 : 2)
zx4_kernel(const InT* __restrict__ vol, int64_t stride_z, int64_t stride_y,
           const mmx_block* __restrict__ blocks, int64_t slot_elems,
           float* __restrict__ gp, float* __restrict__ gq,
           const v4u* __restrict__ xtab, const v4u* __restrict__ ztab, mmx_zx4_cfg cfg)
{
    using cg = cls4<NKX, LA>;
    using pc = pieces4<InT>;
    constexpr int NKZ = cg::NKZ, NT = cg::NT;
    constexpr bool SPLIT = cg::SPLIT;
    constexpr int kUnit = std::is_same<InT, float>::value ? 512 : 256;
    constexpr bool LO_SCALED = lo_scaled4<InT>::value;
    static_assert(NTW == 1 || (NTW == 2 && Q16 && NKX == 2 && LA == 1), "two tiles per wave: 16-bit tiles, 8 < radius <= 16");
    constexpr bool ZLDS = LA == 1 || Q16;
    constexpr int PF = ZLDS ? ZX6_PF : kPF4;
    const mmx_block bd = blocks[blockIdx.y];
    const int W = bd.nx, nz = bd.nz;
    const int ntx = (W + 15) >> 4;
    const int bx = (int)(blockIdx.x & 7) * (int)(gridDim.x >> 3) + (int)(blockIdx.x >> 3);
    const int gw = bx * 4 + __builtin_amdgcn_readfirstlane((int)(threadIdx.x >> 6));
    const int ntp = (ntx + NTW - 1) / NTW;
    const int y = gw / ntp;
    const int c = (gw - y * ntp) * NTW;
    const int lane = threadIdx.x & 63;
    const int li = lane & 15, kq = lane >> 4;
    [[maybe_unused]] const bool lowk = kq < 2;
    int cw = 0, cz = 0;
    for (int i = 1; i < cfg.ncw; ++i) cw = cfg.wcls[i] == W ? i : cw;
    for (int i = 1; i < cfg.ncz; ++i) cz = cfg.zcls[i] == nz ? i : cz;
    const int ntz = (nz + 15) >> 4;
    const int R = cfg.radius;
    const int u_lo = (R + 15) >> 4;
    const int u_hi = (nz - 16 - R) >> 4;
    const v4u* zt = ztab + ((size_t)cz * cfg.maxu * NKZ * 2) * 128 + lane;
    constexpr bool ROT = ZLDS && Q16 && NTW == 1 && !is_f32_4<InT>::value && (NKX == 1 || LA == 2);
    constexpr int ZL1 = NKZ * 4 * 64;
    __shared__ v4u zl[ZLDS ? (ROT ? 2 : 1) * ZL1 : 1];
    if constexpr (ZLDS) {
        const v4u* zi = ztab + ((size_t)(cz * cfg.maxu + (u_lo < cfg.maxu ? u_lo : 0)) * NKZ * 2) * 128;
        for (int e = threadIdx.x; e < ZL1; e += 256) zl[e] = zi[e];
        __syncthreads();
        if constexpr (ROT) {
            for (int e = threadIdx.x; e < ZL1; e += 256) {
                const v4u cur = zl[e];
                const v4u prev = SPLIT ? zl[(e + ZL1 - 256) % ZL1] : (e >= 256 ? zl[e - 256] : (v4u){0u, 0u, 0u, 0u});
                zl[ZL1 + e] = (v4u){prev.z, prev.w, cur.x, cur.y};
            }
            __syncthreads();
        }
    }
    if (y >= bd.ny) return;

    v4u xw[NTW][NKX][2][2];
    const bool has2 = NTW == 2 && c + 1 < ntx;
#pragma unroll
    for (int i = 0; i < NTW; ++i) {
        const v4u* xt = xtab + ((size_t)(cw * cfg.maxcol + (i && !has2 ? c : c + i)) * NKX * 2) * 128 + lane;
#pragma unroll
        for (int m = 0; m < NKX; ++m)
#pragma unroll
            for (int k = 0; k < 2; ++k) {
                xw[i][m][k][0] = xt[(m * 2 + k) * 128];
                xw[i][m][k][1] = xt[(m * 2 + k) * 128 + 64];
            }
    }
    constexpr bool BIASED = Q16 && !is_f32_4<InT>::value && LA == 1;
    constexpr bool MIXSPLIT = Q16;
    const v4f zero4 = {0.f, 0.f, 0.f, 0.f};
    v4f a_start[NTW], b_start[NTW];
#pragma unroll
    for (int i = 0; i < NTW; ++i) { a_start[i] = zero4; b_start[i] = zero4; }
    if constexpr (BIASED) {
        const v4u ones = {0x3C003C00u, 0x3C003C00u, 0x3C003C00u, 0x3C003C00u};
#pragma unroll
        for (int i = 0; i < NTW; ++i) {
            v4f sh[2] = {zero4, zero4}, sl[2] = {zero4, zero4};
#pragma unroll
            for (int m = 0; m < NKX; ++m)
#pragma unroll
                for (int k = 0; k < 2; ++k) {
                    sh[k] = mfma16(ones, xw[i][m][k][0], sh[k]);
                    sl[k] = mfma16(ones, xw[i][m][k][1], sl[k]);
                }
            const float ca = -((pc::kBiasHi + pc::kBiasLo) * sh[0][0] + pc::kBiasHi * sl[0][0] * kLoInv);
            const float cb = -((pc::kBiasHi + pc::kBiasLo) * sh[1][0] + pc::kBiasHi * sl[1][0] * kLoInv);
            a_start[i] = (v4f){ca, ca, ca, ca};
            b_start[i] = (v4f){cb, cb, cb, cb};
        }
    }
    v4u zw[ZLDS ? 1 : NKZ][2][2];
    int zset = -1;

    const InT* in = vol + (int64_t)bd.slot * stride_z;
    const int nch8 = (W + 7) >> 3;
    unsigned xoff[NKX];
#pragma unroll
    for (int m = 0; m < NKX; ++m) {
        int j = 2 * c - cg::R8 / 8 + 4 * m + kq;
        j = j < 0 ? 0 : (j > nch8 - 1 ? nch8 - 1 : j);
        xoff[m] = (unsigned)(j * kUnit + li * 16);
    }
    const rsrc_t rin = make_rsrc(in);
    auto load_tile = [&](int t, typename pc::raw_t (&raw)[NKX]) __attribute__((always_inline)) {
        const unsigned so = (unsigned)((y * ntz + t) * nch8) * (unsigned)kUnit;
#pragma unroll
        for (int m = 0; m < NKX; ++m) raw[m] = pc::load(rin, xoff[m], so);
    };

    unsigned win[NTW][4][NT][2];
#pragma unroll
    for (int w = 0; w < NTW; ++w)
#pragma unroll
        for (int a = 0; a < 4; ++a)
#pragma unroll
            for (int i = 0; i < NT; ++i) { win[w][a][i][0] = 0u; win[w][a][i][1] = 0u; }

    const unsigned col_b = (unsigned)ntz * 1024u;
    const unsigned live_b = col_b - (unsigned)(16 * ntz - nz) * 64u;
    const int64_t wave_e = (int64_t)((y * ntx + c) * ntz) * 256;
    const rsrc_t rp = __builtin_amdgcn_make_buffer_rsrc(gp + (int64_t)bd.slot * slot_elems + wave_e, 0, (int)live_b, 0x00020000);
    const rsrc_t rq = __builtin_amdgcn_make_buffer_rsrc(gq + (int64_t)bd.slot * slot_elems + wave_e, 0, (int)live_b, 0x00020000);
    const rsrc_t rp2 = __builtin_amdgcn_make_buffer_rsrc(gp + (int64_t)bd.slot * slot_elems + wave_e + (int64_t)ntz * 256, 0,
                                                          has2 ? (int)live_b : 0, 0x00020000);
    const unsigned plane_b = 64u;
    unsigned obase = (unsigned)((4 * li + kq) * 16);

    typename pc::raw_t raw[PF][NKX];
#pragma unroll
    for (int u = 0; u < PF; ++u) load_tile(u < ntz ? u : ntz - 1, raw[u]);

    v4f outP[PF][NTW], outQ[PF];
#pragma unroll
    for (int u = 0; u < PF; ++u) {
#pragma unroll
        for (int w = 0; w < NTW; ++w) outP[u][w] = zero4;
        outQ[u] = zero4;
    }
    auto step = [&](int t, auto steady_tag, auto phase_tag, typename pc::raw_t (&rw)[NKX], v4f (&P)[NTW], v4f& Q) __attribute__((always_inline)) {
        constexpr bool STEADY = decltype(steady_tag)::value;
        constexpr int PH = decltype(phase_tag)::value;
        constexpr bool TURN = STEADY && ROT && PH >= 0;
        constexpr int SLOT = TURN ? PH : 2 * LA;
        constexpr int VS = TURN ? PH : 0;
        unsigned xr[4][2] = {{0u, 0u}, {0u, 0u}, {0u, 0u}, {0u, 0u}};
        auto put = [&](int w, int a, int d, unsigned v) __attribute__((always_inline)) {
            if constexpr (SPLIT) xr[a][d] = v;
            else win[w][a][SLOT][d] = v;
        };
        if constexpr (!TURN && !SPLIT) {
#pragma unroll
            for (int w = 0; w < NTW; ++w)
#pragma unroll
                for (int a = 0; a < 4; ++a)
#pragma unroll
                    for (int i = 0; i < 2 * LA; ++i) { win[w][a][i][0] = win[w][a][i + 1][0]; win[w][a][i][1] = win[w][a][i + 1][1]; }
        }
        if (STEADY || t < ntz) {
            v4u dh[NKX], dl[NKX];
#pragma unroll
            for (int m = 0; m < NKX; ++m) {
                if constexpr (BIASED) pc::split_biased(rw[m], dh[m], dl[m]);
                else pc::split(rw[m], dh[m], dl[m]);
            }
            __builtin_amdgcn_sched_barrier(0);
            if (STEADY) load_tile(t + PF < ntz ? t + PF : ntz - 1, rw);
            else if (t + PF < ntz) load_tile(t + PF, rw);
            __builtin_amdgcn_sched_barrier(0);
#pragma unroll
            for (int w = 0; w < NTW; ++w) {
                v4f a0 = a_start[w], a1 = zero4, b0 = b_start[w], b1 = zero4;
#pragma unroll
                for (int m = 0; m < NKX; ++m) {
                    a0 = mfma16(dh[m], xw[w][m][0][0], a0);
                    b0 = mfma16(dh[m], xw[w][m][1][0], b0);
                    a1 = mfma16(dh[m], xw[w][m][0][1], a1);
                    b1 = mfma16(dh[m], xw[w][m][1][1], b1);
                    if constexpr (LO_SCALED) {
                        a1 = mfma16(dl[m], xw[w][m][0][0], a1);
                        b1 = mfma16(dl[m], xw[w][m][1][0], b1);
                    } else {
                        a0 = mfma16(dl[m], xw[w][m][0][0], a0);
                        b0 = mfma16(dl[m], xw[w][m][1][0], b0);
                        if constexpr (!Q16) {
                            a1 = mfma16(dl[m], xw[w][m][0][1], a1);
                            b1 = mfma16(dl[m], xw[w][m][1][1], b1);
                        }
                    }
                }
#pragma unroll
                for (int r = 0; r < 4; r += 2) {
                    const float av0 = __builtin_fmaf(a1[r], kLoInv, a0[r]), av1 = __builtin_fmaf(a1[r + 1], kLoInv, a0[r + 1]);
                    const float bv0 = __builtin_fmaf(b1[r], kLoInv, b0[r]), bv1 = __builtin_fmaf(b1[r + 1], kLoInv, b0[r + 1]);
                    const v2f av = {av0, av1}, bv = {bv0, bv1};
                    const v2h ah = __builtin_convertvector(av, v2h), bh = __builtin_convertvector(bv, v2h);
                    if constexpr (MIXSPLIT) {
                        const v2f ar = {av0 - (float)ah.x, av1 - (float)ah.y}, br = {bv0 - (float)bh.x, bv1 - (float)bh.y};
                        put(w, 0, r >> 1, __builtin_bit_cast(unsigned, ah));
                        put(w, 1, r >> 1, __builtin_bit_cast(unsigned, __builtin_convertvector(ar, v2h)));
                        put(w, 2, r >> 1, __builtin_bit_cast(unsigned, bh));
                        put(w, 3, r >> 1, __builtin_bit_cast(unsigned, __builtin_convertvector(br, v2h)));
                        continue;
                    }
                    const v2f ar = {__builtin_fmaf((float)ah.x, -kLoScale, av0 * kLoScale), __builtin_fmaf((float)ah.y, -kLoScale, av1 * kLoScale)};
                    const v2f br = {__builtin_fmaf((float)bh.x, -kLoScale, bv0 * kLoScale), __builtin_fmaf((float)bh.y, -kLoScale, bv1 * kLoScale)};
                    put(w, 0, r >> 1, __builtin_bit_cast(unsigned, ah));
                    put(w, 1, r >> 1, __builtin_bit_cast(unsigned, __builtin_convertvector(ar, v2h)));
                    put(w, 2, r >> 1, __builtin_bit_cast(unsigned, bh));
                    put(w, 3, r >> 1, __builtin_bit_cast(unsigned, __builtin_convertvector(br, v2h)));
                }
            }
        } else {
#pragma unroll
            for (int w = 0; w < NTW; ++w)
#pragma unroll
                for (int a = 0; a < 4; ++a) { put(w, a, 0, 0u); put(w, a, 1, 0u); }
        }
        const int U = t - LA;
        if (STEADY || U >= 0) {
            const int want = (U >= u_lo && U <= u_hi) ? u_lo : U;
            if constexpr (!STEADY && !ZLDS) {
                if (want != zset) {
                    zset = want;
#pragma unroll
                    for (int ks = 0; ks < NKZ; ++ks)
#pragma unroll
                        for (int k = 0; k < 2; ++k) {
                            zw[ks][k][0] = zt[((size_t)(want * NKZ + ks) * 2 + k) * 128];
                            zw[ks][k][1] = zt[((size_t)(want * NKZ + ks) * 2 + k) * 128 + 64];
                        }
                }
            }
            unsigned vsel[4][2];
#pragma unroll
            for (int a = 0; a < 4; ++a) {
                vsel[a][0] = SPLIT ? (lowk ? xr[a][0] : win[0][a][VS][0]) : 0u;
                vsel[a][1] = SPLIT ? (lowk ? xr[a][1] : win[0][a][VS][1]) : 0u;
            }
            auto wv = [&](int w, int a, int s, int d) __attribute__((always_inline)) {
                return SPLIT && s == VS ? vsel[a][d] : win[w][a][s][d];
            };
            v4f p0[NTW], p1[NTW], q0[NTW], q1[NTW];
#pragma unroll
            for (int w = 0; w < NTW; ++w) { p0[w] = zero4; p1[w] = zero4; q0[w] = zero4; q1[w] = zero4; }
#pragma unroll
            for (int ks = 0; ks < NKZ; ++ks) {
                v4u z00, z01, z10, z11;
                if constexpr (!ZLDS) {
                    z00 = zw[ks][0][0]; z01 = zw[ks][0][1]; z10 = zw[ks][1][0]; z11 = zw[ks][1][1];
                } else if constexpr (STEADY) {
                    constexpr int TR = TURN ? (SPLIT ? PH : (PH - (NT - 2) + NT) % NT) : 0;
                    const int KF = ((TR & 1) ? ZL1 : 0) + ((ks - TR / 2 + NKZ) % NKZ) * 256;
                    z00 = zl[KF + 0 * 64 + lane]; z01 = zl[KF + 1 * 64 + lane];
                    z10 = zl[KF + 2 * 64 + lane]; z11 = zl[KF + 3 * 64 + lane];
                } else {
                    const v4u* zp = zt + ((size_t)(want * NKZ + ks) * 2) * 128;
                    z00 = zp[0]; z01 = zp[64]; z10 = zp[128]; z11 = zp[192];
                }
#pragma unroll
                for (int w = 0; w < NTW; ++w) {
                    const v4u ah = {wv(w, 0, 2 * ks, 0), wv(w, 0, 2 * ks, 1), wv(w, 0, 2 * ks + 1, 0), wv(w, 0, 2 * ks + 1, 1)};
                    const v4u al = {wv(w, 1, 2 * ks, 0), wv(w, 1, 2 * ks, 1), wv(w, 1, 2 * ks + 1, 0), wv(w, 1, 2 * ks + 1, 1)};
                    const v4u bh = {wv(w, 2, 2 * ks, 0), wv(w, 2, 2 * ks, 1), wv(w, 2, 2 * ks + 1, 0), wv(w, 2, 2 * ks + 1, 1)};
                    const v4u bl = {wv(w, 3, 2 * ks, 0), wv(w, 3, 2 * ks, 1), wv(w, 3, 2 * ks + 1, 0), wv(w, 3, 2 * ks + 1, 1)};
                    p0[w] = mfma16(ah, z00, p0[w]);
                    q0[w] = mfma16(bh, z00, q0[w]);
                    p1[w] = mfma16(ah, z01, p1[w]);
                    q1[w] = mfma16(bh, z01, q1[w]);
                    if constexpr (MIXSPLIT) {
                        p0[w] = mfma16(al, z00, p0[w]);
                        q0[w] = mfma16(bl, z00, q0[w]);
                    } else {
                        p1[w] = mfma16(al, z00, p1[w]);
                        q1[w] = mfma16(bl, z00, q1[w]);
                    }
                    q0[w] = mfma16(ah, z10, q0[w]);
                    q1[w] = mfma16(ah, z11, q1[w]);
                    if constexpr (MIXSPLIT) q0[w] = mfma16(al, z10, q0[w]);
                    else q1[w] = mfma16(al, z10, q1[w]);
                }
                if constexpr (ZLDS && !STEADY) __builtin_amdgcn_sched_barrier(0);
            }
            __builtin_amdgcn_sched_barrier(0);
#pragma unroll
            for (int w = 0; w < NTW; ++w) asm volatile("" ::"v"(P[w]));
            if constexpr (!(Q16 && SPLIT)) asm volatile("" ::"v"(Q));
            {
                if constexpr (Q16) {
#pragma unroll
                    for (int w = 0; w < NTW; ++w) {
#pragma unroll
                        for (int r = 0; r < 4; r += 2) {
                            const float pa = __builtin_fmaf(p1[w][r], kLoInv, p0[w][r]), pb = __builtin_fmaf(p1[w][r + 1], kLoInv, p0[w][r + 1]);
                            const float qa = __builtin_fmaf(q1[w][r], kLoInv, q0[w][r]), qb = __builtin_fmaf(q1[w][r + 1], kLoInv, q0[w][r + 1]);
                            const unsigned pu = __builtin_bit_cast(unsigned, __builtin_amdgcn_cvt_pknorm_u16(pa, pb));
                            const unsigned qs = __builtin_bit_cast(unsigned, __builtin_amdgcn_cvt_pknorm_i16(qa, qb));
                            const unsigned da = __builtin_amdgcn_perm(qs, pu, 0x05040100u);
                            const unsigned db = __builtin_amdgcn_perm(qs, pu, 0x07060302u);
                            float ra, rb;
                            asm volatile("v_mov_b32 %0, %1" : "=v"(ra) : "v"(__uint_as_float(da)));
                            asm volatile("v_mov_b32 %0, %1" : "=v"(rb) : "v"(__uint_as_float(db)));
                            P[w][r] = ra;
                            P[w][r + 1] = rb;
                        }
                        if (w == 0) __builtin_amdgcn_raw_buffer_store_b128(__builtin_bit_cast(v4u, P[w]), rp, obase, 0, ZX4_ST_AUX);
                        else __builtin_amdgcn_raw_buffer_store_b128(__builtin_bit_cast(v4u, P[w]), rp2, obase, 0, ZX4_ST_AUX);
                    }
                } else {
#pragma unroll
                for (int r = 0; r < 4; ++r) {
                    const float pv = __builtin_fmaf(p1[0][r], kLoInv, p0[0][r]);
                    const float qv = __builtin_fmaf(q1[0][r], kLoInv, q0[0][r]);
                    float pr, qr;
                    asm volatile("v_mov_b32 %0, %1" : "=v"(pr) : "v"(pv));
                    asm volatile("v_mov_b32 %0, %1" : "=v"(qr) : "v"(qv));
                    P[0][r] = pr;
                    Q[r] = qr;
                }
                __builtin_amdgcn_raw_buffer_store_b128(__builtin_bit_cast(v4u, P[0]), rp, obase, 0, ZX4_ST_AUX);
                __builtin_amdgcn_raw_buffer_store_b128(__builtin_bit_cast(v4u, Q), rq, obase, 0, ZX4_ST_AUX);
                }
            }
            obase += 16u * plane_b;
        }
        if constexpr (SPLIT) {
            if constexpr (!TURN) {
#pragma unroll
                for (int a = 0; a < 4; ++a)
#pragma unroll
                    for (int i = 0; i < NT - 1; ++i) { win[0][a][i][0] = win[0][a][i + 1][0]; win[0][a][i][1] = win[0][a][i + 1][1]; }
            }
#pragma unroll
            for (int a = 0; a < 4; ++a) { win[0][a][TURN ? PH : NT - 1][0] = xr[a][0]; win[0][a][TURN ? PH : NT - 1][1] = xr[a][1]; }
        }
        __builtin_amdgcn_sched_barrier(0);
    };
    const int t_end = ntz + LA;
    int tA = ((u_lo + LA + PF - 1) / PF) * PF;
    int nB = (u_hi + LA + 1 < ntz ? u_hi + LA + 1 : ntz) - tA;
    constexpr int GROUP = ROT ? NT : PF;
    static_assert(GROUP % PF == 0, "a turn of the window is a whole number of rings");
    nB = nB > 0 ? (nB / GROUP) * GROUP : 0;
    if (tA > t_end) tA = ((t_end + PF - 1) / PF) * PF;
    const int tB = tA + nB;
#pragma unroll 1
    for (int t0 = 0; t0 < tA; t0 += PF) {
#pragma unroll
        for (int u = 0; u < PF; ++u)
            if (t0 + u < t_end) step(t0 + u, std::false_type{}, std::integral_constant<int, -1>{}, raw[u], outP[u], outQ[u]);
    }
    if (nB > 0) {
        if (!ZLDS && zset != u_lo) {
            zset = u_lo;
#pragma unroll
            for (int ks = 0; ks < NKZ; ++ks)
#pragma unroll
                for (int k = 0; k < 2; ++k) {
                    zw[ks][k][0] = zt[((size_t)(u_lo * NKZ + ks) * 2 + k) * 128];
                    zw[ks][k][1] = zt[((size_t)(u_lo * NKZ + ks) * 2 + k) * 128 + 64];
                }
        }
        __builtin_amdgcn_s_waitcnt(0x0F70);
        auto turn = [&](int t0, auto... J) __attribute__((always_inline)) {
            (step(t0 + decltype(J)::value, std::true_type{},
                  std::integral_constant<int, ROT ? ((SPLIT ? 0 : NT - 1) + decltype(J)::value) % NT : -1>{},
                  raw[decltype(J)::value % PF], outP[decltype(J)::value % PF], outQ[decltype(J)::value % PF]), ...);
        };
        if constexpr (!ROT) {
#pragma unroll 1
            for (int t0 = tA; t0 < tB; t0 += PF) {
#pragma unroll
                for (int u = 0; u < PF; ++u) step(t0 + u, std::true_type{}, std::integral_constant<int, -1>{}, raw[u], outP[u], outQ[u]);
            }
        } else {
#pragma unroll 1
            for (int t0 = tA; t0 < tB; t0 += GROUP) {
                using std::integral_constant;
                turn(t0, integral_constant<int, 0>{}, integral_constant<int, 1>{}, integral_constant<int, 2>{}, integral_constant<int, 3>{});
                static_assert(GROUP == 4, "a turn is four steps in every class");
            }
        }
    }
#pragma unroll 1
    for (int t0 = tB; t0 < t_end; t0 += PF) {
#pragma unroll
        for (int u = 0; u < PF; ++u)
            if (t0 + u < t_end) step(t0 + u, std::false_type{}, std::integral_constant<int, -1>{}, raw[u], outP[u], outQ[u]);
    }
}



template <typename InT, bool WIDE>
__global__ void __launch_bounds__(256)
zx6_pack_kernel(const InT* __restrict__ vol, int64_t stride_z, int64_t stride_y, int64_t stride_x,
                const mmx_block* __restrict__ blocks, uint16_t* __restrict__ pack, int64_t pack_stride)
{
    constexpr int PITCH = 512 + 8;
    __shared__ __attribute__((aligned(16))) uint16_t tile[16][PITCH];
    const mmx_block bd = blocks[blockIdx.y];
    const int ntz = (bd.nz + 15) >> 4, nrow8 = (bd.nx + 7) >> 3;
    const int yt = blockIdx.x;
    if (yt >= bd.ny * ntz) return;
    const int y = yt / ntz, t = yt - y * ntz;
    const int wave = threadIdx.x >> 6, lane = threadIdx.x & 63;
    const InT* src0 = vol + bd.src_off + (int64_t)y * stride_y;
    bool quads = false;
    if constexpr (sizeof(InT) == 2)
        quads = stride_x == 1 && ((bd.src_off | stride_y | stride_z) & 3) == 0 && (reinterpret_cast<uintptr_t>(vol) & 7) == 0;
    auto panel = [&](int p) __attribute__((always_inline)) {
        const int x0 = WIDE ? 512 * p : 0;
        const int nch8 = WIDE ? (nrow8 - 64 * p < 64 ? nrow8 - 64 * p : 64) : nrow8;
        const int nx = bd.nx - x0;
        const InT* src = src0 + (int64_t)x0 * stride_x;
        if (quads) {
            v2u v[4][2];
            bool have[4][2];
#pragma unroll
            for (int i = 0; i < 4; ++i) {
                const int z = 16 * t + 4 * wave + i;
                const InT* row = src + (int64_t)(z < bd.nz ? z : 0) * stride_z;
#pragma unroll
                for (int h = 0; h < 2; ++h) {
                    const int x = lane * 4 + 256 * h;
                    have[i][h] = x < 8 * nch8;
                    v[i][h] = (v2u){0u, 0u};
                    if (have[i][h] && z < bd.nz) {
                        if (x + 3 < nx) {
                            v[i][h] = *reinterpret_cast<const v2u*>(row + x);
                        } else {
                            unsigned e[4];
#pragma unroll
                            for (int j = 0; j < 4; ++j) e[j] = x + j < nx ? (unsigned)row[x + j] : 0u;
                            v[i][h] = (v2u){e[0] | (e[1] << 16), e[2] | (e[3] << 16)};
                        }
                    }
                }
            }
#pragma unroll
            for (int i = 0; i < 4; ++i)
#pragma unroll
                for (int h = 0; h < 2; ++h)
                    if (have[i][h]) *reinterpret_cast<v2u*>(&tile[4 * wave + i][lane * 4 + 256 * h]) = v[i][h];
        } else
#pragma unroll
        for (int i = 0; i < 4; ++i) {
            const int r = 4 * wave + i, z = 16 * t + r;
            if (z >= bd.nz) {
                for (int x = lane * 4; x < 8 * nch8; x += 256) *reinterpret_cast<v2u*>(&tile[r][x]) = (v2u){0u, 0u};
            } else {
                for (int x = lane; x < 8 * nch8; x += 64)
                    tile[r][x] = x < nx ? (uint16_t)((unsigned)src[(int64_t)z * stride_z + (int64_t)x * stride_x] << (sizeof(InT) == 1 ? 8 : 0))
                                           : (uint16_t)0;
            }
        }
        __syncthreads();
        v4u* dst = reinterpret_cast<v4u*>(pack + (int64_t)bd.slot * pack_stride) + (int64_t)yt * nrow8 * 16 + (WIDE ? 1024 * p : 0);
        for (int u = threadIdx.x; u < nch8 * 16; u += 256) {
            const int j = u >> 4, r = u & 15;
            dst[u] = *reinterpret_cast<const v4u*>(&tile[r][8 * j]);
        }
    };
    if constexpr (WIDE) {
#pragma unroll 1
        for (int p = 0; p < (nrow8 + 63) >> 6; ++p) {
            if (p) __syncthreads();
            panel(p);
        }
    } else {
        panel(0);
    }
}

template <bool WIDE>
__global__ void __launch_bounds__(256)
zx6_pack_f32_kernel(const float* __restrict__ vol, int64_t stride_z, int64_t stride_y, int64_t stride_x,
                    const mmx_block* __restrict__ blocks, uint16_t* __restrict__ pack, int64_t pack_stride)
{
    constexpr int PITCH = 512 + 4;
    __shared__ __attribute__((aligned(16))) unsigned tile[16][PITCH];
    const mmx_block bd = blocks[blockIdx.y];
    const int ntz = (bd.nz + 15) >> 4, nrow8 = (bd.nx + 7) >> 3;
    const int yt = blockIdx.x;
    if (yt >= bd.ny * ntz) return;
    const int y = yt / ntz, t = yt - y * ntz;
    const int wave = threadIdx.x >> 6, lane = threadIdx.x & 63;
    const float* src0 = vol + bd.src_off + (int64_t)y * stride_y;
    auto pieces = [](float v) __attribute__((always_inline)) {
        const _Float16 h = (_Float16)v;
        const _Float16 l = (_Float16)((v - (float)h) * kLoScale);
        return (unsigned)__builtin_bit_cast(unsigned short, h) | ((unsigned)__builtin_bit_cast(unsigned short, l) << 16);
    };
    const bool quads = stride_x == 1 && ((bd.src_off | stride_y | stride_z) & 3) == 0 && (reinterpret_cast<uintptr_t>(vol) & 15) == 0;
    auto panel = [&](int p) __attribute__((always_inline)) {
        const int x0 = WIDE ? 512 * p : 0;
        const int nch8 = WIDE ? (nrow8 - 64 * p < 64 ? nrow8 - 64 * p : 64) : nrow8;
        const int nx = bd.nx - x0;
        const float* src = src0 + (int64_t)x0 * stride_x;
#pragma unroll
        for (int i = 0; i < 4; ++i) {
            const int r = 4 * wave + i, z = 16 * t + r;
            if (quads && z < bd.nz) {
                const float* row = src + (int64_t)z * stride_z;
                for (int x = lane * 4; x < 8 * nch8; x += 256) {
                    v4f v = {0.f, 0.f, 0.f, 0.f};
                    if (x + 3 < nx) v = *reinterpret_cast<const v4f*>(row + x);
                    else
                        for (int j = 0; j < 4; ++j) v[j] = x + j < nx ? row[x + j] : 0.f;
                    *reinterpret_cast<v4u*>(&tile[r][x]) = (v4u){pieces(v[0]), pieces(v[1]), pieces(v[2]), pieces(v[3])};
                }
            } else {
                for (int x = lane; x < 8 * nch8; x += 64) {
                    float v = 0.f;
                    if (z < bd.nz && x < nx) v = src[(int64_t)z * stride_z + (int64_t)x * stride_x];
                    tile[r][x] = pieces(v);
                }
            }
        }
        __syncthreads();
        v4u* dst = reinterpret_cast<v4u*>(pack + (int64_t)bd.slot * pack_stride) + (int64_t)yt * nrow8 * 32 + (WIDE ? 2048 * p : 0);
        for (int u = threadIdx.x; u < nch8 * 16; u += 256) {
            const int j = u >> 4, r = u & 15;
            const v4u a = *reinterpret_cast<const v4u*>(&tile[r][8 * j]);
            const v4u b = *reinterpret_cast<const v4u*>(&tile[r][8 * j + 4]);
            const v4u hi = {__builtin_amdgcn_perm(a[1], a[0], 0x05040100u), __builtin_amdgcn_perm(a[3], a[2], 0x05040100u),
                             __builtin_amdgcn_perm(b[1], b[0], 0x05040100u), __builtin_amdgcn_perm(b[3], b[2], 0x05040100u)};
            const v4u lo = {__builtin_amdgcn_perm(a[1], a[0], 0x07060302u), __builtin_amdgcn_perm(a[3], a[2], 0x07060302u),
                             __builtin_amdgcn_perm(b[1], b[0], 0x07060302u), __builtin_amdgcn_perm(b[3], b[2], 0x07060302u)};
            dst[j * 32 + r] = hi;
            dst[j * 32 + 16 + r] = lo;
        }
    };
    if constexpr (WIDE) {
#pragma unroll 1
        for (int p = 0; p < (nrow8 + 63) >> 6; ++p) {
            if (p) __syncthreads();
            panel(p);
        }
    } else {
        panel(0);
    }
}

struct zx_classes {
    int ncw, ncz, wcls[MMX_ZX4_MAXCLS], zcls[MMX_ZX4_MAXCLS];
    int maxcol, maxu;
};
bool collect_classes(const mmx_block* h_blocks, int n_blocks, zx_classes* c)
{
    c->ncw = c->ncz = c->maxcol = c->maxu = 0;
    for (int i = 0; i < n_blocks; ++i) {
        const mmx_block& b = h_blocks[i];
        int j;
        for (j = 0; j < c->ncw && c->wcls[j] != b.nx; ++j) {}
        if (j == c->ncw) { if (j == MMX_ZX4_MAXCLS) return false; c->wcls[c->ncw++] = b.nx; }
        for (j = 0; j < c->ncz && c->zcls[j] != b.nz; ++j) {}
        if (j == c->ncz) { if (j == MMX_ZX4_MAXCLS) return false; c->zcls[c->ncz++] = b.nz; }
        c->maxcol = std::max(c->maxcol, (b.nx + 15) / 16);
        c->maxu = std::max(c->maxu, (b.nz + 15) / 16);
    }
    return true;
}

template <int NKX, int LA>
int launch_zx6(const mmx_volume* vol, const mmx_block* d_blocks, const mmx_block* h_blocks, int n_blocks,
               const mmx_zx6_plan& plan, const mmx_taps_f32& tx, int radius, void* d_work, float qp, float qq, hipStream_t s)
{
    using cg = cls4<NKX, LA>;
    mmx_zx4_cfg cfg{};
    for (int k = 0; k <= MMX_MAX_RADIUS_FAST; ++k) { cfg.w0[k] = tx.w0[k]; cfg.w2[k] = tx.w2[k]; }
    cfg.radius = radius;
    cfg.xscale = vol->dtype == MMX_U16 ? (float)(65536.0 / 65535.0) :
                 (vol->dtype == MMX_U8 ? (float)(65536.0 / (255.0 * 256.0)) : 1.f);
    cfg.staged = 2;
    cfg.qp = qp; cfg.qq = qq;
    const bool pair = NKX == 2 && LA == 1 && qp > 0.f && vol->dtype != MMX_F32;
    cfg.ntw = pair ? 2 : 1;
    zx_classes cl;
    if (!collect_classes(h_blocks, n_blocks, &cl)) return MMX_ERR_UNSUPPORTED;
    cfg.ncw = cl.ncw; cfg.ncz = cl.ncz; cfg.maxcol = cl.maxcol; cfg.maxu = cl.maxu;
    for (int j = 0; j < MMX_ZX4_MAXCLS; ++j) {
        cfg.wcls[j] = j < cl.ncw ? cl.wcls[j] : -1;
        cfg.zcls[j] = j < cl.ncz ? cl.zcls[j] : -1;
    }
    int max_waves = 0;
    for (int i = 0; i < n_blocks; ++i) {
        const mmx_block& b = h_blocks[i];
        if (!mmx_zx6_launch_accepts(vol, b.nz, b.nx, radius)) return MMX_ERR_UNSUPPORTED;
        const int ntx = (b.nx + 15) / 16;
        max_waves = std::max(max_waves, b.ny * (pair ? (ntx + 1) / 2 : ntx));
    }
    const int nx_entries = cfg.ncw * cfg.maxcol * NKX * 2;
    const int nz_entries = cfg.ncz * cfg.maxu * cg::NKZ * 2;
    const size_t xbytes = (size_t)nx_entries * 2 * 64 * sizeof(v4u);
    const size_t zbytes = (size_t)nz_entries * 2 * 64 * sizeof(v4u);
    if ((int64_t)(xbytes + zbytes) > plan.tab_bytes) return MMX_ERR_UNSUPPORTED;
    char* w = reinterpret_cast<char*>(d_work);
    v4u* xtab = reinterpret_cast<v4u*>(w + plan.tab_off);
    v4u* ztab = reinterpret_cast<v4u*>(w + plan.tab_off + xbytes);
    hipLaunchKernelGGL((zx4_setup<NKX, LA>), dim3((nx_entries + nz_entries + 3) / 4), dim3(256), 0, s, cfg, xtab, ztab);
    dim3 grid((((max_waves + 3) / 4) + 7) & ~7, n_blocks);
    if (vol->dtype == MMX_F32) {
        if (qp > 0.f)
            hipLaunchKernelGGL((zx4_kernel<NKX, LA, float, true>), grid, dim3(256), 0, s,
                               reinterpret_cast<const float*>(w + plan.pack_off), plan.pack_stride / 2, (int64_t)0, d_blocks,
                               plan.tile_stride, reinterpret_cast<float*>(w), reinterpret_cast<float*>(w + plan.q_off),
                               xtab, ztab, cfg);
        else
            hipLaunchKernelGGL((zx4_kernel<NKX, LA, float, false>), grid, dim3(256), 0, s,
                               reinterpret_cast<const float*>(w + plan.pack_off), plan.pack_stride / 2, (int64_t)0, d_blocks,
                               plan.tile_stride, reinterpret_cast<float*>(w), reinterpret_cast<float*>(w + plan.q_off),
                               xtab, ztab, cfg);
    } else if (pair) {
        if constexpr (NKX == 2 && LA == 1)
            hipLaunchKernelGGL((zx4_kernel<NKX, LA, uint16_t, true, 2>), grid, dim3(256), 0, s,
                               reinterpret_cast<const uint16_t*>(w + plan.pack_off), plan.pack_stride, (int64_t)0, d_blocks,
                               plan.tile_stride, reinterpret_cast<float*>(w), reinterpret_cast<float*>(w + plan.q_off),
                               xtab, ztab, cfg);
    } else if (qp > 0.f)
        hipLaunchKernelGGL((zx4_kernel<NKX, LA, uint16_t, true>), grid, dim3(256), 0, s,
                           reinterpret_cast<const uint16_t*>(w + plan.pack_off), plan.pack_stride, (int64_t)0, d_blocks,
                           plan.tile_stride, reinterpret_cast<float*>(w), reinterpret_cast<float*>(w + plan.q_off),
                           xtab, ztab, cfg);
    else
        hipLaunchKernelGGL((zx4_kernel<NKX, LA, uint16_t, false>), grid, dim3(256), 0, s,
                           reinterpret_cast<const uint16_t*>(w + plan.pack_off), plan.pack_stride, (int64_t)0, d_blocks,
                           plan.tile_stride, reinterpret_cast<float*>(w), reinterpret_cast<float*>(w + plan.q_off),
                           xtab, ztab, cfg);
    return hipGetLastError() == hipSuccess ? MMX_OK : MMX_ERR_HIP;
}

}

int mmx_zx6_plan_make(const mmx_block* h_blocks, int n_blocks, int64_t slot_elems, int voxel_dtype, mmx_zx6_plan* plan)
{
    const int pieces = voxel_dtype == MMX_F32 ? 2 : 1;
    int64_t tile = 0, pk = 0;
    int max_tiles = 0, max_rowtiles = 0;
    zx_classes cl;
    if (!collect_classes(h_blocks, n_blocks, &cl)) return MMX_ERR_UNSUPPORTED;
    for (int i = 0; i < n_blocks; ++i) {
        const mmx_block& b = h_blocks[i];
        const int ntx = (b.nx + 15) / 16, ntz = (b.nz + 15) / 16, nch8 = (b.nx + 7) / 8;
        const int64_t te = (int64_t)ntx * ntz * b.ny * 256, pe = (int64_t)b.ny * ntz * nch8 * 128 * pieces;
        if (te > tile) tile = te;
        if (pe > pk) pk = pe;
        if (ntx * ntz > max_tiles) max_tiles = ntx * ntz;
        if (b.ny * ntz > max_rowtiles) max_rowtiles = b.ny * ntz;
    }
    if (tile * 4 >= (int64_t(1) << 31) || pk * 2 >= (int64_t(1) << 31)) return MMX_ERR_UNSUPPORTED;
    plan->tile_stride = tile;
    plan->pack_stride = pk;
    plan->q_off = (int64_t)n_blocks * tile * 4;
    plan->tab_off = 2 * plan->q_off;
    plan->tab_bytes = (int64_t)(cl.ncw * cl.maxcol * 2 * 2 + cl.ncz * cl.maxu * 3 * 2) * 2 * 64 * 16;
    plan->pack_off = (plan->tab_off + plan->tab_bytes + 255) & ~int64_t(255);
    plan->max_tiles = max_tiles;
    plan->max_rowtiles = max_rowtiles;
    const int64_t need = plan->pack_off + (int64_t)n_blocks * pk * 2;
    return need <= 4 * (int64_t)n_blocks * slot_elems * 4 ? MMX_OK : MMX_ERR_UNSUPPORTED;
}

int mmx_launch_zx6_pack(const mmx_volume* vol, const mmx_block* d_blocks, const mmx_block* h_blocks, int n_blocks,
                        const mmx_zx6_plan& plan, void* d_work, hipStream_t stream)
{
    if (!mmx_voxels_ok(vol)) return MMX_ERR_UNSUPPORTED;
    uint16_t* pack = reinterpret_cast<uint16_t*>(reinterpret_cast<char*>(d_work) + plan.pack_off);
    dim3 grid(plan.max_rowtiles, n_blocks);
    bool wide = false;
    for (int i = 0; i < n_blocks; ++i) wide = wide || h_blocks[i].nx > 512;
    auto launch = [&](auto kernel, auto* data) {
        hipLaunchKernelGGL(kernel, grid, dim3(256), 0, stream, data, vol->stride_z, vol->stride_y, vol->stride_x, d_blocks, pack,
                           plan.pack_stride);
    };
    if (vol->dtype == MMX_F32) {
        if (wide) launch(zx6_pack_f32_kernel<true>, (const float*)vol->d_data);
        else launch(zx6_pack_f32_kernel<false>, (const float*)vol->d_data);
    } else if (vol->dtype == MMX_U16) {
        if (wide) launch(zx6_pack_kernel<uint16_t, true>, (const uint16_t*)vol->d_data);
        else launch(zx6_pack_kernel<uint16_t, false>, (const uint16_t*)vol->d_data);
    } else {
        if (wide) launch(zx6_pack_kernel<uint8_t, true>, (const uint8_t*)vol->d_data);
        else launch(zx6_pack_kernel<uint8_t, false>, (const uint8_t*)vol->d_data);
    }
    return hipGetLastError() == hipSuccess ? MMX_OK : MMX_ERR_HIP;
}

int mmx_launch_zx6(const mmx_volume* vol, const mmx_block* d_blocks, const mmx_block* h_blocks, int n_blocks,
                   const mmx_zx6_plan& plan, const mmx_taps_f32& tx, int radius, void* d_work, float qp, float qq,
                   hipStream_t stream)
{
    if (!mmx_ring_radius(radius) || !mmx_voxels_ok(vol)) return MMX_ERR_UNSUPPORTED;
    if (radius <= 8) return launch_zx6<1, 1>(vol, d_blocks, h_blocks, n_blocks, plan, tx, radius, d_work, qp, qq, stream);
    if (radius <= 16) return launch_zx6<2, 1>(vol, d_blocks, h_blocks, n_blocks, plan, tx, radius, d_work, qp, qq, stream);
    return launch_zx6<2, 2>(vol, d_blocks, h_blocks, n_blocks, plan, tx, radius, d_work, qp, qq, stream);
}
```

magellanmapper_amd/csrc/mmx_route.h:

```cpp
#pragma once

#include <cmath>
#include <cstddef>
#include <vector>

#define MMX_PACKED_MAX_PX 320
#define MMX_YM_MAX_RADIUS 24
#define MMX_X_OUTPUTS 8
#define MMX_X_MAX_QUADS 2
#define MMX_X_MAX_HALO 2
#define MMX_X_THREADS 256
#define MMX_LDS_BYTES (64 * 1024)

struct mmx_zx_request { int mode; bool y_valu, prepacked; };
inline int mmx_zx_parse(int zx_mode, mmx_zx_request* q)
{
    q->y_valu = zx_mode >= 0 && (zx_mode & MMX_ZX_Y_VALU);
    if (q->y_valu) zx_mode &= ~MMX_ZX_Y_VALU;
    q->prepacked = zx_mode == (MMX_ZX_TILED | MMX_ZX_PREPACKED) || zx_mode == (MMX_ZX_TILED_Q16 | MMX_ZX_PREPACKED);
    if (q->prepacked) zx_mode &= ~MMX_ZX_PREPACKED;
    q->mode = zx_mode;
    if (zx_mode < MMX_ZX_AUTO || zx_mode > MMX_ZX_THIN || zx_mode == 1 || (zx_mode >= 3 && zx_mode <= 5))
        return MMX_ERR_ARG;
    return MMX_OK;
}

inline bool mmx_voxels_ok(const mmx_volume* vol) { return vol->dtype == MMX_U8 || vol->dtype == MMX_U16 || vol->dtype == MMX_F32; }
inline bool mmx_ring_radius(int radius) { return radius >= 1 && radius <= MMX_MAX_RADIUS_FAST; }
inline bool mmx_lane_ok(const mmx_volume* vol, const mmx_batch_geom& g)
{
    return g.max_lane_in * 8 < (int64_t(1) << 31) && vol->stride_y < (1 << 30);
}

inline bool mmx_wide_launch_accepts(const mmx_volume* vol, int radius)
{
    return radius >= 1 && radius <= MMX_MAX_RADIUS_WIDE && mmx_voxels_ok(vol);
}
inline bool mmx_wide_accepts(const mmx_volume* vol, const mmx_batch_geom& g, int radius)
{
    return mmx_wide_launch_accepts(vol, radius) && g.status == MMX_OK && g.min_nz >= radius && g.min_ny >= radius && g.min_nx >= radius;
}

inline bool mmx_zpass_accepts(const mmx_volume* vol, const mmx_batch_geom& g, int radius)
{
    return mmx_ring_radius(radius) && mmx_voxels_ok(vol) && mmx_lane_ok(vol, g) && g.min_nz >= radius + MMX_COL_PREFETCH;
}
inline bool mmx_ypass_accepts(const mmx_batch_geom& g, int radius)
{
    return mmx_ring_radius(radius) && g.min_ny >= radius + MMX_COL_PREFETCH;
}
struct mmx_xpass_shape { int px, pw, ch, rg; size_t lds_bytes; };
inline mmx_xpass_shape mmx_xpass_shape_of(int max_nx, int R)
{
    mmx_xpass_shape x;
    const int lead = R & 1, s = (R + lead + 7) & ~7;
    x.px = (max_nx + MMX_ROW_ALIGN - 1) / MMX_ROW_ALIGN * MMX_ROW_ALIGN;
    const int span = s + x.px + R + lead;
    x.pw = ((span + 2 * (span >> 3)) + 3) & ~1;
    x.ch = (max_nx + MMX_X_OUTPUTS - 1) / MMX_X_OUTPUTS;
    x.rg = x.ch > 0 ? MMX_X_THREADS / x.ch : 1;
    if (x.rg < 1) x.rg = 1;
    while (x.rg > 1 && (x.rg * (x.px / 4) > MMX_X_MAX_QUADS * MMX_X_THREADS || x.rg * 2 * R > MMX_X_MAX_HALO * MMX_X_THREADS)) --x.rg;
    x.lds_bytes = ((size_t)2 * x.rg * x.pw + (size_t)x.rg * x.px) * sizeof(float);
    return x;
}
inline bool mmx_xpass_launch_accepts(int max_nx, int radius)
{
    if (!mmx_ring_radius(radius) || max_nx < 1) return false;
    const mmx_xpass_shape x = mmx_xpass_shape_of(max_nx, radius);
    if (x.px / 4 > MMX_X_MAX_QUADS * MMX_X_THREADS || 2 * radius > MMX_X_MAX_HALO * MMX_X_THREADS) return false;
    if (x.ch > MMX_X_THREADS) return false;
    return x.lds_bytes <= MMX_LDS_BYTES;
}
inline bool mmx_xpass_accepts(const mmx_batch_geom& g, int radius)
{
    return g.min_nx >= radius && mmx_xpass_launch_accepts(g.max_nx, radius);
}

inline bool mmx_thin_accepts(const mmx_batch_geom& g, int radius)
{
    const int thin_below = radius + MMX_COL_PREFETCH;
    return radius >= 0 && radius <= MMX_MAX_RADIUS_GENERIC && g.status == MMX_OK &&
           (g.min_nz < thin_below || g.min_ny < thin_below || g.min_nx < thin_below);
}

inline bool mmx_fused_accepts(const mmx_volume* vol, const mmx_batch_geom& g, int radius)
{
    return mmx_ring_radius(radius) && mmx_lane_ok(vol, g) && g.min_ny >= radius + MMX_COL_PREFETCH && g.min_nz >= radius + 1 &&
           g.min_nx >= radius;
}
inline bool mmx_zx2_launch_accepts(const mmx_volume* vol, int max_px, int radius)
{
    return mmx_ring_radius(radius) && mmx_voxels_ok(vol) && max_px <= MMX_PACKED_MAX_PX &&
           vol->stride_z * 8 * (int64_t)sizeof(double) < (int64_t(1) << 32);
}
inline bool mmx_packed_accepts(const mmx_volume* vol, const mmx_batch_geom& g, int radius)
{
    return mmx_fused_accepts(vol, g, radius) && mmx_zx2_launch_accepts(vol, g.max_px, radius);
}
inline bool mmx_zx6_launch_accepts(const mmx_volume* vol, int min_nz, int min_nx, int radius)
{
    return mmx_ring_radius(radius) && mmx_voxels_ok(vol) && min_nx >= radius && min_nz >= radius;
}
inline bool mmx_tiled_accepts(const mmx_volume* vol, const mmx_batch_geom& g, int radius)
{
    return mmx_fused_accepts(vol, g, radius) && g.plan_status == MMX_OK && mmx_zx6_launch_accepts(vol, g.min_nz, g.min_nx, radius);
}
inline bool mmx_ym_accepts(const float* w0, const float* w2, int radius, float cp, float cq)
{
    if (radius < 1 || radius > MMX_YM_MAX_RADIUS || radius > MMX_MAX_RADIUS_FAST || !(cp > 0.f) || !(cq > 0.f)) return false;
    float mx = 0.f;
    for (int k = 0; k <= radius; ++k) mx = fmaxf(mx, fmaxf(fabsf(w2[k] * cp), fabsf(w0[k] * cq)));
    return mx > 1e-30f && mx < 1e30f;
}

inline void mmx_q16_bounds(const double* w0, const double* w2, int radius, double norm, double* bp, double* bq, double* err)
{
    double s0 = w0[0], s2 = fabs(w2[0]);
    for (int k = 1; k <= radius; ++k) { s0 += 2.0 * w0[k]; s2 += 2.0 * fabs(w2[k]); }
    *bp = s0 * s0 * (1.0 + 1e-6);
    double pos = 0.0, neg = 0.0;
    for (int i = 0; i <= radius; ++i)
        for (int j = 0; j <= radius; ++j) {
            const double k = (w2[i] * w0[j] + w0[i] * w2[j]) * ((i ? 2.0 : 1.0) * (j ? 2.0 : 1.0));
            if (k > 0.0) pos += k; else neg -= k;
        }
    *bq = (pos > neg ? pos : neg) * (1.0 + 1e-4);
    const double drop = 255.0 / 65536.0 / 2048.0;
    const double biased = 4.0 * 0x1p-22;
    const double ydrop = 255.0 / 4096.0;
    *err = norm * (s2 * (*bp / 65535.0 * (0.5 + ydrop) + drop * s0 * s0 + biased * *bp) +
                   s0 * (*bq / 32767.0 * (0.5 + ydrop) + drop * 2.0 * s2 * s0 + biased * *bq)) + 1e-6;
}
inline double mmx_q16_error_bound(const double* w0, const double* w2, int radius, double norm)
{
    if (!w0 || !w2 || radius < 0 || radius > MMX_MAX_RADIUS_GENERIC) return -1.0;
    double bp, bq, err;
    mmx_q16_bounds(w0, w2, radius, norm, &bp, &bq, &err);
    return err;
}

inline bool mmx_tiles_q16(int zx_mode, const mmx_volume* vol, double unit_bound, double band, bool entries, double* value_scale)
{
    const bool ranged = vol->dtype == MMX_F32 && vol->value_range > 0.f && vol->value_range < 60000.f;
    *value_scale = vol->dtype == MMX_U8 || vol->dtype == MMX_U16 ? 1.0 : (ranged ? (double)vol->value_range : 0.0);
    if (!(*value_scale > 0.0)) return false;
    if (zx_mode == MMX_ZX_TILED_Q16) return true;
    const double bound = unit_bound * *value_scale;
    return zx_mode == MMX_ZX_AUTO && entries && bound >= 0.0 && 4.0 * bound <= band && bound <= MMX_LOG_ABS_TOL;
}

enum mmx_route_family { MMX_ROUTE_SEPARATE = 0, MMX_ROUTE_WIDE, MMX_ROUTE_TILED, MMX_ROUTE_PACKED };
enum mmx_route_y { MMX_Y_NONE = 0, MMX_Y_YM, MMX_Y_Y6, MMX_Y_Y2 };
struct mmx_route {
    int family;
    bool q16;
    bool makes_copy;
    bool trusts_copy;
    int y_kernel;
    bool ring_z, ring_y, ring_x;
    bool fold_z, fold_y, fold_x;
    int layout;
    int path;
    double bp, bq;
};

inline int mmx_route_scale(const mmx_volume* vol, const mmx_batch_geom& g, int radius, const double* w0, const double* w2,
                           double norm, int zx_mode, double band, bool entries, mmx_route* r, int thin_radius = -1)
{
    *r = mmx_route{};
    r->path = MMX_ZX_SEPARATE;
    mmx_zx_request q;
    if (mmx_zx_parse(zx_mode, &q) != MMX_OK || radius < 0) return MMX_ERR_ARG;
    if (radius > MMX_MAX_RADIUS_GENERIC || !mmx_voxels_ok(vol)) return MMX_ERR_UNSUPPORTED;
    if (g.status != MMX_OK) return g.status;
    if (q.mode == MMX_ZX_THIN) {
        if (mmx_thin_accepts(g, thin_radius < 0 ? radius : thin_radius)) {
            r->family = MMX_ROUTE_SEPARATE;
            r->path = MMX_ZX_THIN;
            r->ring_z = mmx_zpass_accepts(vol, g, radius);
            r->ring_y = mmx_ypass_accepts(g, radius);
            r->ring_x = mmx_xpass_accepts(g, radius);
            r->fold_z = !r->ring_z;
            r->fold_y = !r->ring_y;
            r->fold_x = !r->ring_x;
            return MMX_OK;
        }
        q.mode = MMX_ZX_AUTO;
    }
    if ((q.mode == MMX_ZX_WIDE || (q.mode == MMX_ZX_AUTO && radius > MMX_MAX_RADIUS_FAST)) && mmx_wide_accepts(vol, g, radius)) {
        r->family = MMX_ROUTE_WIDE;
        r->path = MMX_ZX_WIDE;
        r->layout = entries && g.rows_fit ? MMX_MASK_ROWS : 0;
        return MMX_OK;
    }
    if (q.mode != MMX_ZX_SEPARATE && mmx_fused_accepts(vol, g, radius)) {
        const bool integer = vol->dtype == MMX_U8 || vol->dtype == MMX_U16;
        const bool ranged = vol->dtype == MMX_F32 && vol->value_range != 0.f && fabsf(vol->value_range) < 60000.f;
        double bp, bq, err, vscale;
        mmx_q16_bounds(w0, w2, radius, norm, &bp, &bq, &err);
        const bool q16 = mmx_tiles_q16(q.mode, vol, err, band, entries, &vscale);
        const bool named = q.mode == MMX_ZX_TILED || (q.mode == MMX_ZX_TILED_Q16 && vscale > 0.0);
        if ((named || (q.mode == MMX_ZX_AUTO && (integer || ranged))) && mmx_tiled_accepts(vol, g, radius)) {
            r->family = MMX_ROUTE_TILED;
            r->q16 = q16;
            r->trusts_copy = q.prepacked;
            r->makes_copy = !q.prepacked;
            r->path = q16 ? MMX_ZX_TILED_Q16 : MMX_ZX_TILED;
            r->layout = entries && g.quads_fit ? MMX_MASK_QUADS : 0;
            r->y_kernel = MMX_Y_Y6;
            if (q16) {
                r->bp = bp * vscale;
                r->bq = bq * vscale;
                float y0[MMX_MAX_RADIUS_FAST + 1], y2[MMX_MAX_RADIUS_FAST + 1];
                for (int k = 0; k <= radius; ++k) { y0[k] = (float)(-norm * w0[k]); y2[k] = (float)(-norm * w2[k]); }
                if (!q.y_valu && mmx_ym_accepts(y0, y2, radius, (float)(r->bp / 65535.0), (float)(r->bq / 32767.0)))
                    r->y_kernel = MMX_Y_YM;
            }
            return MMX_OK;
        }
        if (mmx_packed_accepts(vol, g, radius)) {
            r->family = MMX_ROUTE_PACKED;
            r->path = MMX_ZX_PACKED;
            r->layout = entries && g.rows_fit ? MMX_MASK_ROWS : 0;
            r->y_kernel = MMX_Y_Y2;
            return MMX_OK;
        }
    }
    r->family = MMX_ROUTE_SEPARATE;
    r->ring_z = mmx_zpass_accepts(vol, g, radius);
    r->ring_y = mmx_ypass_accepts(g, radius);
    r->ring_x = mmx_xpass_accepts(g, radius);
    return MMX_OK;
}

struct mmx_ladder_route {
    int n_configs;
    int layout;
    int zx_path;
    double q16_bound;
    bool copy;
    bool copy_on_side;
};

inline int mmx_route_config(const mmx_volume* vol, const mmx_batch_geom& g, const int32_t* radii, const double* w0_tab,
                            const double* w2_tab, const double* norms, int n_sigma, int mode, int zx_flags,
                            const int32_t* modes, double band, bool entries, mmx_route* routes, mmx_ladder_route* out,
                            int thin_radius = -1)
{
    const size_t tab = MMX_MAX_RADIUS_GENERIC + 1;
    const bool is_float = vol->dtype == MMX_F32;
    const bool float_ok = is_float && vol->value_range != 0.f;
    int tiled_mode = MMX_ZX_TILED;
    double q16_bound = 0.0;
    if (mode == MMX_ZX_AUTO || mode == MMX_ZX_TILED_Q16) {
        double bound = 0.0;
        for (int s = 0; s < n_sigma; ++s) {
            const double b = mmx_q16_error_bound(w0_tab + s * tab, w2_tab + s * tab, radii[s], norms[s]);
            if (b < 0) { bound = -1.0; break; }
            if (b > bound) bound = b;
        }
        double vscale;
        if (mmx_tiles_q16(mode, vol, bound, band, true, &vscale)) { tiled_mode = MMX_ZX_TILED_Q16; q16_bound = bound * vscale; }
    }
    const bool may_tile = ((mode == MMX_ZX_AUTO || mode == MMX_ZX_TILED || mode == MMX_ZX_TILED_Q16) && !is_float) ||
                          ((mode == MMX_ZX_AUTO || mode == MMX_ZX_TILED) && float_ok);
    out->copy = !modes && may_tile && mmx_voxels_ok(vol) && !g.bad_block && g.plan_status == MMX_OK;
    bool trusted = out->copy;
    int layouts = 0;
    for (int s = 0; s < n_sigma; ++s) {
        const int m = modes ? modes[s] : (trusted ? (tiled_mode | MMX_ZX_PREPACKED | zx_flags) : mode);
        const int rc = mmx_route_scale(vol, g, radii[s], w0_tab + s * tab, w2_tab + s * tab, norms[s], m, band, entries, &routes[s],
                                       thin_radius);
        if (rc != MMX_OK) return -rc;
        trusted = trusted && routes[s].path == tiled_mode;
        layouts |= 1 << routes[s].layout;
        out->zx_path = routes[s].path;
    }
    out->q16_bound = !modes && out->zx_path == MMX_ZX_TILED_Q16 ? q16_bound : 0.0;
    return layouts;
}

inline int mmx_route_ladder(const mmx_volume* vol, const mmx_batch_geom& g, const int32_t* radii, const double* w0_tab,
                            const double* w2_tab, const double* norms, int n_sigma, int zx_mode, int zx_flags, double band,
                            mmx_route* routes, mmx_ladder_route* out)
{
    *out = mmx_ladder_route{};
    int layouts = 0;
    auto config = [&](int mode, const int32_t* modes, bool entries) {
        out->n_configs++;
        layouts = mmx_route_config(vol, g, radii, w0_tab, w2_tab, norms, n_sigma, mode, zx_flags, modes, band, entries, routes, out);
        return layouts < 0 || !(layouts & (layouts - 1));
    };
    if (zx_mode == MMX_ZX_THIN) {
        int r_max = 0;
        for (int s = 0; s < n_sigma; ++s) if (radii[s] > r_max) r_max = radii[s];
        if (!mmx_thin_accepts(g, r_max)) zx_mode = MMX_ZX_AUTO;
        else {
            out->n_configs = 1;
            layouts = mmx_route_config(vol, g, radii, w0_tab, w2_tab, norms, n_sigma, zx_mode, zx_flags, nullptr, band, false,
                                       routes, out, r_max);
            if (layouts < 0) return -layouts;
            return MMX_OK;
        }
    }
    bool any_wide = false;
    if (zx_mode == MMX_ZX_AUTO && g.status == MMX_OK)
        for (int s = 0; s < n_sigma; ++s)
            if (radii[s] > MMX_MAX_RADIUS_FAST && mmx_wide_accepts(vol, g, radii[s])) any_wide = true;
    if (any_wide) {
        std::vector<int32_t> laid(n_sigma);
        int32_t* modes = laid.data();
        bool entries = g.rows_fit;
        for (int s = 0; s < n_sigma; ++s) {
            const int r = radii[s];
            if (r <= MMX_MAX_RADIUS_FAST && mmx_packed_accepts(vol, g, r)) modes[s] = MMX_ZX_PACKED;
            else if (mmx_wide_accepts(vol, g, r)) modes[s] = MMX_ZX_WIDE;
            else { modes[s] = MMX_ZX_AUTO; entries = false; }
        }
        if (!config(MMX_ZX_AUTO, modes, entries)) {
            for (int s = 0; s < n_sigma; ++s) modes[s] = MMX_ZX_AUTO;
            config(MMX_ZX_AUTO, modes, false);
        }
    } else if (!config(zx_mode, nullptr, true)) {
        if (layouts != ((1 << MMX_MASK_ROWS) | (1 << MMX_MASK_QUADS)) || !config(MMX_ZX_PACKED, nullptr, true))
            config(zx_mode, nullptr, false);
    }
    if (layouts < 0) return -layouts;
    out->layout = 0;
    while (!(layouts & (1 << out->layout))) ++out->layout;
    out->copy_on_side = out->copy && out->n_configs == 1;
    return MMX_OK;
}
```

Baseline: 45030.

## Stage z-edge tap tiles in LDS and issue first voxel loads early in zx4

Adds an LDS-resident variant of the tiled zx4 MFMA kernel for 16-bit quantised integer volumes. It copies the boundary (edge) z-tap tiles into shared memory alongside the interior set, and replaces the branchy head/tail loop with fixed-form edge steps that read taps from LDS. The first prefetch-ring voxel loads are issued before the x-tap setup so their latency overlaps it. This costs more LDS per block, which may lower occupancy, and a new flag keeps the old global-table edge path available.

```diff
diff --git a/include/mmx.h b/include/mmx.h
--- a/include/mmx.h
+++ b/include/mmx.h
@@ -75,6 +75,7 @@
 } mmx_zx_mode;
 #define MMX_ZX_PREPACKED 0x100
 #define MMX_ZX_Y_VALU    0x200
+#define MMX_ZX_EDGE_GLOBAL 0x400
 #define MMX_MASK_ROWS 1
 #define MMX_MASK_QUADS 2
 int mmx_log_batch_f32(const mmx_volume* vol, const mmx_block* d_blocks, const mmx_block* h_blocks,
diff --git a/magellanmapper_amd/_native.py b/magellanmapper_amd/_native.py
--- a/magellanmapper_amd/_native.py
+++ b/magellanmapper_amd/_native.py
@@ -20,6 +20,7 @@
 MMX_CAND_PROBE = 4
 MMX_ZX_AUTO, MMX_ZX_SEPARATE, MMX_ZX_PACKED, MMX_ZX_MFMA_F32, MMX_ZX_MFMA_F16, MMX_ZX_MFMA_F16_LDS = -1, 0, 2, 3, 4, 5
 MMX_ZX_TILED, MMX_ZX_TILED_Q16, MMX_ZX_PREPACKED, MMX_ZX_Y_VALU = 6, 7, 0x100, 0x200
+MMX_ZX_EDGE_GLOBAL = 0x400
 MMX_ZX_WIDE = 8
 MMX_ZX_THIN = 9
 MMX_FOLD_MAX_N = 68
diff --git a/magellanmapper_amd/csrc/mmx_api.hip b/magellanmapper_amd/csrc/mmx_api.hip
--- a/magellanmapper_amd/csrc/mmx_api.hip
+++ b/magellanmapper_amd/csrc/mmx_api.hip
@@ -267,7 +267,7 @@
     { mmx_timed_scope ts(MMX_K_ZX, s);
       if (tiled)
           rc = mmx_launch_zx6(vol, c.d_blocks, c.h_blocks, n_blocks, plan, txx, radius, c.d_work,
-                              r.q16 ? (float)(1.0 / r.bp) : 0.f, r.q16 ? (float)(1.0 / r.bq) : 0.f, s);
+                              r.q16 ? (float)(1.0 / r.bp) : 0.f, r.q16 ? (float)(1.0 / r.bq) : 0.f, r.edge_global, s);
       else
           rc = mmx_launch_zx2(vol, c.d_blocks, n_blocks, g.max_ny, g.max_px, slot_elems, tzz, txx, radius, t0, t1, s); }
     if (rc != MMX_OK) return launched(rc, tiled ? "mmx_launch_zx6" : "mmx_launch_zx2", "fused passes");
diff --git a/magellanmapper_amd/csrc/mmx_common.h b/magellanmapper_amd/csrc/mmx_common.h
--- a/magellanmapper_amd/csrc/mmx_common.h
+++ b/magellanmapper_amd/csrc/mmx_common.h
@@ -48,7 +48,7 @@
                         const mmx_zx6_plan& plan, void* d_work, hipStream_t stream);
 int mmx_launch_zx6(const mmx_volume* vol, const mmx_block* d_blocks, const mmx_block* h_blocks, int n_blocks,
                    const mmx_zx6_plan& plan, const mmx_taps_f32& tx, int radius, void* d_work, float qp, float qq,
-                   hipStream_t stream);
+                   bool edge_global, hipStream_t stream);
 int mmx_launch_y6(const mmx_block* d_blocks, int n_blocks, const mmx_zx6_plan& plan, int64_t slot_elems,
                   const mmx_taps_f32& taps, int radius, const float* d_p, const float* d_q, float cp, float cq,
                   float* d_log, unsigned long long* d_mask, float nms_lo, float nms_eps, hipStream_t stream);
diff --git a/magellanmapper_amd/csrc/mmx_fused4.hip b/magellanmapper_amd/csrc/mmx_fused4.hip
--- a/magellanmapper_amd/csrc/mmx_fused4.hip
+++ b/magellanmapper_amd/csrc/mmx_fused4.hip
@@ -49,7 +49,27 @@
     static constexpr bool SPLIT = LA == 2;
     static constexpr int NKZ = 2;
     static constexpr int NT = 4;
+    static constexpr int kMaxEdge = LA == 1 ? 3 : 4;
 };
+
+struct zx4_edges { int u_lo, u_hi, hi0, n; };
+__host__ __device__ inline zx4_edges zx4_edge_tiles(int nz, int R)
+{
+    zx4_edges e;
+    const int ntz = (nz + 15) >> 4;
+    e.u_lo = (R + 15) >> 4;
+    e.u_hi = (nz - 16 - R) >> 4;
+    e.hi0 = e.u_hi + 1 > e.u_lo ? e.u_hi + 1 : e.u_lo;
+    e.n = e.u_lo + (ntz > e.hi0 ? ntz - e.hi0 : 0);
+    return e;
+}
+template <int NKX, int LA>
+bool zx4_edges_fit(int nz, int R)
+{
+    const zx4_edges e = zx4_edge_tiles(nz, R);
+    const int ntz = (nz + 15) >> 4;
+    return e.n <= cls4<NKX, LA>::kMaxEdge && e.u_lo == LA && ntz + LA >= 2 * LA && ntz >= e.u_lo;
+}
 
 __device__ __forceinline__ float folded_tap(const float* w, int R, int p, int o, int n)
 {
@@ -179,7 +199,7 @@
 template <typename InT> struct lo_scaled4 { static constexpr bool value = false; };
 template <> struct lo_scaled4<float> { static constexpr bool value = true; };
 
-template <int NKX, int LA, typename InT, bool Q16 = false, int NTW = 1>
+template <int NKX, int LA, typename InT, bool Q16 = false, int NTW = 1, bool ELDS = false>
 __global__ void __launch_bounds__(256, (NTW == 1 && (LA == 1 || Q16) && !is_f32_4<InT>::value) ? 3 : 2)
 zx4_kernel(const InT* __restrict__ vol, int64_t stride_z, int64_t stride_y,
            const mmx_block* __restrict__ blocks, int64_t slot_elems,
@@ -216,10 +236,32 @@
     const v4u* zt = ztab + ((size_t)cz * cfg.maxu * NKZ * 2) * 128 + lane;
     constexpr bool ROT = ZLDS && Q16 && NTW == 1 && !is_f32_4<InT>::value && (NKX == 1 || LA == 2);
     constexpr int ZL1 = NKZ * 4 * 64;
-    __shared__ v4u zl[ZLDS ? (ROT ? 2 : 1) * ZL1 : 1];
+    constexpr bool EDGE = ELDS;
+    static_assert(!ELDS || (ZLDS && Q16 && !is_f32_4<InT>::value), "LDS edge tables: 16-bit tiles of integer voxels");
+    constexpr int MAXE = EDGE ? cg::kMaxEdge : 0;
+    constexpr int ZE0 = (ROT ? 2 : 1) * ZL1;
+    const int hi0 = zx4_edge_tiles(nz, R).hi0;
+    __shared__ v4u zl[ZLDS ? ZE0 + MAXE * ZL1 : 1];
     if constexpr (ZLDS) {
         const v4u* zi = ztab + ((size_t)(cz * cfg.maxu + (u_lo < cfg.maxu ? u_lo : 0)) * NKZ * 2) * 128;
-        for (int e = threadIdx.x; e < ZL1; e += 256) zl[e] = zi[e];
+        if constexpr (EDGE) {
+            const v4u* zc = ztab + ((size_t)(cz * cfg.maxu) * NKZ * 2) * 128;
+            v4u f[MAXE + 1][ZL1 / 256];
+#pragma unroll
+            for (int sl = 0; sl <= MAXE; ++sl) {
+                int tile = sl - 1 < u_lo ? sl - 1 : hi0 + (sl - 1 - u_lo);
+                tile = tile < ntz - 1 ? tile : ntz - 1;
+                const v4u* src = sl ? zc + ((size_t)tile * NKZ * 2) * 128 : zi;
+#pragma unroll
+                for (int j = 0; j < ZL1 / 256; ++j) f[sl][j] = src[threadIdx.x + 256 * j];
+            }
+#pragma unroll
+            for (int sl = 0; sl <= MAXE; ++sl)
+#pragma unroll
+                for (int j = 0; j < ZL1 / 256; ++j) zl[(sl ? ZE0 + (sl - 1) * ZL1 : 0) + threadIdx.x + 256 * j] = f[sl][j];
+        } else {
+            for (int e = threadIdx.x; e < ZL1; e += 256) zl[e] = zi[e];
+        }
         __syncthreads();
         if constexpr (ROT) {
             for (int e = threadIdx.x; e < ZL1; e += 256) {
@@ -231,6 +273,23 @@
         }
     }
     if (y >= bd.ny) return;
+
+    [[maybe_unused]] typename pc::raw_t raw_early[ELDS ? PF : 1][NKX];
+    if constexpr (ELDS) {
+        const rsrc_t rin0 = make_rsrc(vol + (int64_t)bd.slot * stride_z);
+        const int nch0 = (W + 7) >> 3;
+#pragma unroll
+        for (int u = 0; u < PF; ++u) {
+            const unsigned so = (unsigned)((y * ntz + (u < ntz ? u : ntz - 1)) * nch0) * (unsigned)kUnit;
+#pragma unroll
+            for (int m = 0; m < NKX; ++m) {
+                int j = 2 * c - cg::R8 / 8 + 4 * m + kq;
+                j = j < 0 ? 0 : (j > nch0 - 1 ? nch0 - 1 : j);
+                raw_early[u][m] = pc::load(rin0, (unsigned)(j * kUnit + li * 16), so);
+            }
+        }
+        __builtin_amdgcn_sched_barrier(0);
+    }
 
     v4u xw[NTW][NKX][2][2];
     const bool has2 = NTW == 2 && c + 1 < ntx;
@@ -307,8 +366,16 @@
     unsigned obase = (unsigned)((4 * li + kq) * 16);
 
     typename pc::raw_t raw[PF][NKX];
-#pragma unroll
-    for (int u = 0; u < PF; ++u) load_tile(u < ntz ? u : ntz - 1, raw[u]);
+    constexpr bool EARLY = ELDS;
+    if constexpr (EARLY) {
+#pragma unroll
+        for (int u = 0; u < PF; ++u)
+#pragma unroll
+            for (int m = 0; m < NKX; ++m) raw[u][m] = raw_early[u][m];
+    } else {
+#pragma unroll
+        for (int u = 0; u < PF; ++u) load_tile(u < ntz ? u : ntz - 1, raw[u]);
+    }
 
     v4f outP[PF][NTW], outQ[PF];
 #pragma unroll
@@ -317,9 +384,12 @@
         for (int w = 0; w < NTW; ++w) outP[u][w] = zero4;
         outQ[u] = zero4;
     }
-    auto step = [&](int t, auto steady_tag, auto phase_tag, typename pc::raw_t (&rw)[NKX], v4f (&P)[NTW], v4f& Q) __attribute__((always_inline)) {
+    auto step = [&](int t, auto steady_tag, auto phase_tag, typename pc::raw_t (&rw)[NKX], v4f (&P)[NTW], v4f& Q,
+                    auto form_tag, int zb) __attribute__((always_inline)) {
         constexpr bool STEADY = decltype(steady_tag)::value;
         constexpr int PH = decltype(phase_tag)::value;
+        constexpr int FORM = decltype(form_tag)::value;
+        constexpr bool NOBR = STEADY || FORM != 0;
         constexpr bool TURN = STEADY && ROT && PH >= 0;
         constexpr int SLOT = TURN ? PH : 2 * LA;
         constexpr int VS = TURN ? PH : 0;
@@ -336,7 +406,7 @@
 #pragma unroll
                     for (int i = 0; i < 2 * LA; ++i) { win[w][a][i][0] = win[w][a][i + 1][0]; win[w][a][i][1] = win[w][a][i + 1][1]; }
         }
-        if (STEADY || t < ntz) {
+        if (NOBR || t < ntz) {
             v4u dh[NKX], dl[NKX];
 #pragma unroll
             for (int m = 0; m < NKX; ++m) {
@@ -344,7 +414,7 @@
                 else pc::split(rw[m], dh[m], dl[m]);
             }
             __builtin_amdgcn_sched_barrier(0);
-            if (STEADY) load_tile(t + PF < ntz ? t + PF : ntz - 1, rw);
+            if (NOBR) load_tile(t + PF < ntz ? t + PF : ntz - 1, rw);
             else if (t + PF < ntz) load_tile(t + PF, rw);
             __builtin_amdgcn_sched_barrier(0);
 #pragma unroll
@@ -397,7 +467,7 @@
                 for (int a = 0; a < 4; ++a) { put(w, a, 0, 0u); put(w, a, 1, 0u); }
         }
         const int U = t - LA;
-        if (STEADY || U >= 0) {
+        if (FORM != 1 && (NOBR || U >= 0)) {
             const int want = (U >= u_lo && U <= u_hi) ? u_lo : U;
             if constexpr (!STEADY && !ZLDS) {
                 if (want != zset) {
@@ -433,6 +503,10 @@
                     const int KF = ((TR & 1) ? ZL1 : 0) + ((ks - TR / 2 + NKZ) % NKZ) * 256;
                     z00 = zl[KF + 0 * 64 + lane]; z01 = zl[KF + 1 * 64 + lane];
                     z10 = zl[KF + 2 * 64 + lane]; z11 = zl[KF + 3 * 64 + lane];
+                } else if constexpr (FORM == 2) {
+                    const int KF = zb + ks * 256 + lane;
+                    z00 = zl[KF + 0 * 64]; z01 = zl[KF + 1 * 64];
+                    z10 = zl[KF + 2 * 64]; z11 = zl[KF + 3 * 64];
                 } else {
                     const v4u* zp = zt + ((size_t)(want * NKZ + ks) * 2) * 128;
                     z00 = zp[0]; z01 = zp[64]; z10 = zp[128]; z11 = zp[192];
@@ -459,7 +533,7 @@
                     if constexpr (MIXSPLIT) q0[w] = mfma16(al, z10, q0[w]);
                     else q1[w] = mfma16(al, z10, q1[w]);
                 }
-                if constexpr (ZLDS && !STEADY) __builtin_amdgcn_sched_barrier(0);
+                if constexpr (ZLDS && !STEADY && FORM == 0) __builtin_amdgcn_sched_barrier(0);
             }
             __builtin_amdgcn_sched_barrier(0);
 #pragma unroll
@@ -503,6 +577,14 @@
             }
             obase += 16u * plane_b;
         }
+        if constexpr (FORM == 1) {
+            constexpr unsigned kDropped = 0x80000000u;
+#pragma unroll
+            for (int w = 0; w < NTW; ++w) {
+                if (w == 0) __builtin_amdgcn_raw_buffer_store_b128(__builtin_bit_cast(v4u, P[w]), rp, kDropped, 0, ZX4_ST_AUX);
+                else __builtin_amdgcn_raw_buffer_store_b128(__builtin_bit_cast(v4u, P[w]), rp2, kDropped, 0, ZX4_ST_AUX);
+            }
+        }
         if constexpr (SPLIT) {
             if constexpr (!TURN) {
 #pragma unroll
@@ -523,11 +605,29 @@
     nB = nB > 0 ? (nB / GROUP) * GROUP : 0;
     if (tA > t_end) tA = ((t_end + PF - 1) / PF) * PF;
     const int tB = tA + nB;
+    [[maybe_unused]] auto edge_step = [&](int t, auto u_tag, auto form_tag, int zb) __attribute__((always_inline)) {
+        constexpr int u = decltype(u_tag)::value;
+        step(t, std::false_type{}, std::integral_constant<int, -1>{}, raw[u], outP[u], outQ[u], form_tag, zb);
+    };
+    if constexpr (EDGE) {
+        using std::integral_constant;
+        static_assert(PF == 2, "the head and tail of the LDS form are written for a ring of two");
+        if constexpr (LA == 1) {
+            edge_step(0, integral_constant<int, 0>{}, integral_constant<int, 1>{}, 0);
+            edge_step(1, integral_constant<int, 1>{}, integral_constant<int, 2>{}, ZE0);
+        } else {
+            edge_step(0, integral_constant<int, 0>{}, integral_constant<int, 1>{}, 0);
+            edge_step(1, integral_constant<int, 1>{}, integral_constant<int, 1>{}, 0);
+            edge_step(2, integral_constant<int, 0>{}, integral_constant<int, 2>{}, ZE0);
+            edge_step(3, integral_constant<int, 1>{}, integral_constant<int, 2>{}, ZE0 + ZL1);
+        }
+    } else {
 #pragma unroll 1
-    for (int t0 = 0; t0 < tA; t0 += PF) {
-#pragma unroll
-        for (int u = 0; u < PF; ++u)
-            if (t0 + u < t_end) step(t0 + u, std::false_type{}, std::integral_constant<int, -1>{}, raw[u], outP[u], outQ[u]);
+        for (int t0 = 0; t0 < tA; t0 += PF) {
+#pragma unroll
+            for (int u = 0; u < PF; ++u)
+                if (t0 + u < t_end) step(t0 + u, std::false_type{}, std::integral_constant<int, -1>{}, raw[u], outP[u], outQ[u], std::integral_constant<int, 0>{}, 0);
+        }
     }
     if (nB > 0) {
         if (!ZLDS && zset != u_lo) {
@@ -540,17 +640,18 @@
                     zw[ks][k][1] = zt[((size_t)(u_lo * NKZ + ks) * 2 + k) * 128 + 64];
                 }
         }
-        __builtin_amdgcn_s_waitcnt(0x0F70);
+        if constexpr (!EDGE) __builtin_amdgcn_s_waitcnt(0x0F70);
         auto turn = [&](int t0, auto... J) __attribute__((always_inline)) {
             (step(t0 + decltype(J)::value, std::true_type{},
                   std::integral_constant<int, ROT ? ((SPLIT ? 0 : NT - 1) + decltype(J)::value) % NT : -1>{},
-                  raw[decltype(J)::value % PF], outP[decltype(J)::value % PF], outQ[decltype(J)::value % PF]), ...);
+                  raw[decltype(J)::value % PF], outP[decltype(J)::value % PF], outQ[decltype(J)::value % PF],
+                  std::integral_constant<int, 0>{}, 0), ...);
         };
         if constexpr (!ROT) {
 #pragma unroll 1
             for (int t0 = tA; t0 < tB; t0 += PF) {
 #pragma unroll
-                for (int u = 0; u < PF; ++u) step(t0 + u, std::true_type{}, std::integral_constant<int, -1>{}, raw[u], outP[u], outQ[u]);
+                for (int u = 0; u < PF; ++u) step(t0 + u, std::true_type{}, std::integral_constant<int, -1>{}, raw[u], outP[u], outQ[u], std::integral_constant<int, 0>{}, 0);
             }
         } else {
 #pragma unroll 1
@@ -561,11 +662,23 @@
             }
         }
     }
+    if constexpr (EDGE) {
+        using std::integral_constant;
+        auto zb_of = [&](int U) __attribute__((always_inline)) { return U <= u_hi ? 0 : ZE0 + (u_lo + U - hi0) * ZL1; };
+        int t0 = tB;
+#pragma unroll 1
+        for (; t0 + PF <= t_end; t0 += PF) {
+            edge_step(t0, integral_constant<int, 0>{}, integral_constant<int, 2>{}, zb_of(t0 - LA));
+            edge_step(t0 + 1, integral_constant<int, 1>{}, integral_constant<int, 2>{}, zb_of(t0 + 1 - LA));
+        }
+        if (t0 < t_end) edge_step(t0, integral_constant<int, 0>{}, integral_constant<int, 2>{}, zb_of(t0 - LA));
+        return;
+    }
 #pragma unroll 1
     for (int t0 = tB; t0 < t_end; t0 += PF) {
 #pragma unroll
         for (int u = 0; u < PF; ++u)
-            if (t0 + u < t_end) step(t0 + u, std::false_type{}, std::integral_constant<int, -1>{}, raw[u], outP[u], outQ[u]);
+            if (t0 + u < t_end) step(t0 + u, std::false_type{}, std::integral_constant<int, -1>{}, raw[u], outP[u], outQ[u], std::integral_constant<int, 0>{}, 0);
     }
 }
 
@@ -744,7 +857,8 @@
 
 template <int NKX, int LA>
 int launch_zx6(const mmx_volume* vol, const mmx_block* d_blocks, const mmx_block* h_blocks, int n_blocks,
-               const mmx_zx6_plan& plan, const mmx_taps_f32& tx, int radius, void* d_work, float qp, float qq, hipStream_t s)
+               const mmx_zx6_plan& plan, const mmx_taps_f32& tx, int radius, void* d_work, float qp, float qq, bool edge_global,
+               hipStream_t s)
 {
     using cg = cls4<NKX, LA>;
     mmx_zx4_cfg cfg{};
@@ -770,6 +884,8 @@
         const int ntx = (b.nx + 15) / 16;
         max_waves = std::max(max_waves, b.ny * (pair ? (ntx + 1) / 2 : ntx));
     }
+    bool elds = NKX == 2 && !edge_global && qp > 0.f && vol->dtype != MMX_F32;
+    for (int j = 0; j < cl.ncz; ++j) elds = elds && zx4_edges_fit<NKX, LA>(cl.zcls[j], radius);
     const int nx_entries = cfg.ncw * cfg.maxcol * NKX * 2;
     const int nz_entries = cfg.ncz * cfg.maxu * cg::NKZ * 2;
     const size_t xbytes = (size_t)nx_entries * 2 * 64 * sizeof(v4u);
@@ -792,17 +908,32 @@
                                plan.tile_stride, reinterpret_cast<float*>(w), reinterpret_cast<float*>(w + plan.q_off),
                                xtab, ztab, cfg);
     } else if (pair) {
-        if constexpr (NKX == 2 && LA == 1)
-            hipLaunchKernelGGL((zx4_kernel<NKX, LA, uint16_t, true, 2>), grid, dim3(256), 0, s,
-                               reinterpret_cast<const uint16_t*>(w + plan.pack_off), plan.pack_stride, (int64_t)0, d_blocks,
-                               plan.tile_stride, reinterpret_cast<float*>(w), reinterpret_cast<float*>(w + plan.q_off),
-                               xtab, ztab, cfg);
-    } else if (qp > 0.f)
-        hipLaunchKernelGGL((zx4_kernel<NKX, LA, uint16_t, true>), grid, dim3(256), 0, s,
-                           reinterpret_cast<const uint16_t*>(w + plan.pack_off), plan.pack_stride, (int64_t)0, d_blocks,
-                           plan.tile_stride, reinterpret_cast<float*>(w), reinterpret_cast<float*>(w + plan.q_off),
-                           xtab, ztab, cfg);
-    else
+        if constexpr (NKX == 2 && LA == 1) {
+            if (elds)
+                hipLaunchKernelGGL((zx4_kernel<NKX, LA, uint16_t, true, 2, true>), grid, dim3(256), 0, s,
+                                   reinterpret_cast<const uint16_t*>(w + plan.pack_off), plan.pack_stride, (int64_t)0, d_blocks,
+                                   plan.tile_stride, reinterpret_cast<float*>(w), reinterpret_cast<float*>(w + plan.q_off),
+                                   xtab, ztab, cfg);
+            else
+                hipLaunchKernelGGL((zx4_kernel<NKX, LA, uint16_t, true, 2>), grid, dim3(256), 0, s,
+                                   reinterpret_cast<const uint16_t*>(w + plan.pack_off), plan.pack_stride, (int64_t)0, d_blocks,
+                                   plan.tile_stride, reinterpret_cast<float*>(w), reinterpret_cast<float*>(w + plan.q_off),
+                                   xtab, ztab, cfg);
+        }
+    } else if (qp > 0.f) {
+        if constexpr (!(NKX == 2 && LA == 1)) {
+            if constexpr (NKX == 2) if (elds)
+                hipLaunchKernelGGL((zx4_kernel<NKX, LA, uint16_t, true, 1, true>), grid, dim3(256), 0, s,
+                                   reinterpret_cast<const uint16_t*>(w + plan.pack_off), plan.pack_stride, (int64_t)0, d_blocks,
+                                   plan.tile_stride, reinterpret_cast<float*>(w), reinterpret_cast<float*>(w + plan.q_off),
+                                   xtab, ztab, cfg);
+            if (!elds)
+                hipLaunchKernelGGL((zx4_kernel<NKX, LA, uint16_t, true>), grid, dim3(256), 0, s,
+                                   reinterpret_cast<const uint16_t*>(w + plan.pack_off), plan.pack_stride, (int64_t)0, d_blocks,
+                                   plan.tile_stride, reinterpret_cast<float*>(w), reinterpret_cast<float*>(w + plan.q_off),
+                                   xtab, ztab, cfg);
+        }
+    } else
         hipLaunchKernelGGL((zx4_kernel<NKX, LA, uint16_t, false>), grid, dim3(256), 0, s,
                            reinterpret_cast<const uint16_t*>(w + plan.pack_off), plan.pack_stride, (int64_t)0, d_blocks,
                            plan.tile_stride, reinterpret_cast<float*>(w), reinterpret_cast<float*>(w + plan.q_off),
@@ -868,10 +999,10 @@
 
 int mmx_launch_zx6(const mmx_volume* vol, const mmx_block* d_blocks, const mmx_block* h_blocks, int n_blocks,
                    const mmx_zx6_plan& plan, const mmx_taps_f32& tx, int radius, void* d_work, float qp, float qq,
-                   hipStream_t stream)
+                   bool edge_global, hipStream_t stream)
 {
     if (!mmx_ring_radius(radius) || !mmx_voxels_ok(vol)) return MMX_ERR_UNSUPPORTED;
-    if (radius <= 8) return launch_zx6<1, 1>(vol, d_blocks, h_blocks, n_blocks, plan, tx, radius, d_work, qp, qq, stream);
-    if (radius <= 16) return launch_zx6<2, 1>(vol, d_blocks, h_blocks, n_blocks, plan, tx, radius, d_work, qp, qq, stream);
-    return launch_zx6<2, 2>(vol, d_blocks, h_blocks, n_blocks, plan, tx, radius, d_work, qp, qq, stream);
-}
+    if (radius <= 8) return launch_zx6<1, 1>(vol, d_blocks, h_blocks, n_blocks, plan, tx, radius, d_work, qp, qq, edge_global, stream);
+    if (radius <= 16) return launch_zx6<2, 1>(vol, d_blocks, h_blocks, n_blocks, plan, tx, radius, d_work, qp, qq, edge_global, stream);
+    return launch_zx6<2, 2>(vol, d_blocks, h_blocks, n_blocks, plan, tx, radius, d_work, qp, qq, edge_global, stream);
+}
diff --git a/magellanmapper_amd/csrc/mmx_route.h b/magellanmapper_amd/csrc/mmx_route.h
--- a/magellanmapper_amd/csrc/mmx_route.h
+++ b/magellanmapper_amd/csrc/mmx_route.h
@@ -12,11 +12,13 @@
 #define MMX_X_THREADS 256
 #define MMX_LDS_BYTES (64 * 1024)
 
-struct mmx_zx_request { int mode; bool y_valu, prepacked; };
+struct mmx_zx_request { int mode; bool y_valu, prepacked, edge_global; };
 inline int mmx_zx_parse(int zx_mode, mmx_zx_request* q)
 {
     q->y_valu = zx_mode >= 0 && (zx_mode & MMX_ZX_Y_VALU);
     if (q->y_valu) zx_mode &= ~MMX_ZX_Y_VALU;
+    q->edge_global = zx_mode >= 0 && (zx_mode & MMX_ZX_EDGE_GLOBAL);
+    if (q->edge_global) zx_mode &= ~MMX_ZX_EDGE_GLOBAL;
     q->prepacked = zx_mode == (MMX_ZX_TILED | MMX_ZX_PREPACKED) || zx_mode == (MMX_ZX_TILED_Q16 | MMX_ZX_PREPACKED);
     if (q->prepacked) zx_mode &= ~MMX_ZX_PREPACKED;
     q->mode = zx_mode;
@@ -157,6 +159,7 @@
     bool q16;
     bool makes_copy;
     bool trusts_copy;
+    bool edge_global;
     int y_kernel;
     bool ring_z, ring_y, ring_x;
     bool fold_z, fold_y, fold_x;
@@ -206,6 +209,7 @@
             r->q16 = q16;
             r->trusts_copy = q.prepacked;
             r->makes_copy = !q.prepacked;
+            r->edge_global = q.edge_global;
             r->path = q16 ? MMX_ZX_TILED_Q16 : MMX_ZX_TILED;
             r->layout = entries && g.quads_fit ? MMX_MASK_QUADS : 0;
             r->y_kernel = MMX_Y_Y6;
```

Measured after the change: 46580, median of 6. +3.4%, better.
